# geekieo/collaborative-deep-metric-learning

Hardware: AMD Instinct MI355X
Metric: triplets/sec (higher is better)
Workload: dtype f32 values as 3 exact bf16 planes (hi + mid + lo == the f32 value), 6 bf16-MFMA plane products per f32 product, f32 accumulate

## Files before the change

__graft_entry__.py:

```python
import glob
import os
import subprocess
import sys

ROOT = os.path.dirname(os.path.abspath(__file__))
PKG = os.path.join(ROOT, "collaborative-deep-metric-learning_amd")
CSRC = os.path.join(PKG, "csrc")
LIB = os.path.join(PKG, "lib", "libcdml_hip.so")
if ROOT not in sys.path:
    sys.path.insert(0, ROOT)


def _stale(target, sources):
    if not os.path.exists(target):
        return True
    t = os.path.getmtime(target)
    return any(os.path.getmtime(s) > t for s in sources)


def _ids():
    import importlib.util
    spec = importlib.util.spec_from_file_location("_cdml_lib_ids", os.path.join(PKG, "_lib.py"))
    m = importlib.util.module_from_spec(spec)
    spec.loader.exec_module(m)
# ... 4 lines not shown
    from concurrent.futures import ThreadPoolExecutor
    os.makedirs(objdir, exist_ok=True)
    jobs = []
    import re
    for s in srcs:
        o = os.path.join(objdir, os.path.basename(s)[:-4] + ".o")
        inc = [os.path.join(os.path.dirname(s), m) for m in re.findall(r'#include "([^"]+\.hip)"', open(s).read())]
        if force or _stale(o, [s] + inc + hdrs):
            jobs.append([hipcc] + flags + ["-c", "-o", o, s])
    if jobs:
        print("[build] compiling %d of %d sources" % (len(jobs), len(srcs)), flush=True)

        def run(c):
            r = subprocess.run(c + ["-Rpass-analysis=kernel-resource-usage"], cwd=CSRC, stderr=subprocess.PIPE, text=True)
            o = c[c.index("-o") + 1]
            with open(o[:-2] + ".remarks", "w") as f:
                f.write(r.stderr)
            if r.returncode:
                sys.stderr.write("\n".join(ln for ln in r.stderr.splitlines() if "remark:" not in ln)[-4000:] + "\n")
            return r
        with ThreadPoolExecutor(max_workers=min(len(jobs), max(1, (os.cpu_count() or 2) - 1))) as ex:
            for r in ex.map(run, jobs):
                if r.returncode:
                    raise RuntimeError("hipcc failed: " + " ".join(r.args))
    objs = [os.path.join(objdir, os.path.basename(s)[:-4] + ".o") for s in srcs]
    _check_no_scratch(objs)
    return objs


NPAIR_KERNELS = ("k_npair", "k_mixed", "k_npdp")


def _check_no_scratch(objs):
    import re
    bad = []
    for o in objs:
        rem = o[:-2] + ".remarks"
        if not os.path.exists(rem):
            continue
        name = None
        for ln in open(rem):
            m = re.search(r"Function Name: (\S+)", ln)
            if m:
                name = m.group(1)
            m = re.search(r"ScratchSize \[bytes/lane\]: (\d+)", ln)
            if m and name and int(m.group(1)) > 0 and any(k in name for k in ("k_gemm",) + NPAIR_KERNELS):
                bad.append("%s: %s bytes of scratch per lane (%s)" % (name, m.group(1), os.path.basename(o)))
    if bad:
        raise RuntimeError("kernels with a scratch frame (GEMMs: spills inside hand-counted vmcnt pipelines; N-pair launches "
                           "(k_npair / k_mixed / k_npdp): spills in bandwidth-bound passes):\n  " + "\n  ".join(bad))


def build(force=False, csrc=None, lib=None, objdir=None):
    variant = csrc is not None
    csrc = csrc or CSRC
    lib = lib or LIB
    objdir = objdir or os.path.join(ROOT, "build", "obj")
    srcs = sorted(glob.glob(os.path.join(csrc, "*.hip")))
    hdrs = glob.glob(os.path.join(csrc, "*.h")) + [os.path.join(ROOT, "include", "cdml.h")] \
        + glob.glob(os.path.join(ROOT, "include", "cdml_*.h"))
    source_id, embedded_id = _ids()
    sid = source_id(csrc, os.path.join(ROOT, "include", "cdml.h"))
    if force or embedded_id(lib) != sid:
        os.makedirs(os.path.dirname(lib), exist_ok=True)
        hipcc = os.environ.get("HIPCC", "/opt/rocm/bin/hipcc")
        flags = ["--offload-arch=gfx950", "-O3", "-std=c++17", "-fPIC", "-I" + CSRC,
                 "-Wno-array-bounds"]
        objs = _compile_objects(srcs, hdrs, objdir, hipcc, flags, force)
        idsrc = os.path.join(objdir, "build_id.cpp")
        with open(idsrc, "w") as f:
            f.write('extern "C" const char *cdml_build_id(void) { return "CDML_BUILD_ID=%s"; }\n' % sid)
        subprocess.run([hipcc, "-O1", "-fPIC", "-c", "-o", idsrc[:-4] + ".o", idsrc], check=True)
        objs.append(idsrc[:-4] + ".o")
        cmd = [hipcc, "--offload-arch=gfx950", "-fPIC", "-shared", "-o", lib] + objs
        print("[build]", " ".join(cmd), flush=True)
        subprocess.run(cmd, check=True, cwd=csrc)
    if variant:
        return
    import cdml_amd
    from cdml_amd import _lib
    lib = _lib.load_library()
    assert lib.cdml_version() >= 1000
    for name in list(_lib.SIGNATURES) + list(_lib.SIGNATURES_MIXED) + list(_lib.SIGNATURES_DP) + list(_lib.SIGNATURES_BF16) \
            + list(_lib.SIGNATURES_HARDNEG):
        getattr(lib, name)
    assert lib.cdml_build_id().decode() == "CDML_BUILD_ID=" + sid
    print("[build] ok:", LIB, "version", lib.cdml_version(), lib.cdml_build_id().decode())


def smoke():
    import numpy as np
    import torch
    build()
    from cdml_amd import engine, train
    from oracle import sampler as osampler, synth as osynth, tower as otower

    dev = torch.device("cuda:0")
    N, F, H, D, B = 512, 96, 200, 32, 128
    table = engine.FeatureTable.synthetic(N, F, seed=0, device=dev)
    feats = osynth.features_philox(0, N, F, 0)
    assert np.array_equal(table.data[:, :F].cpu().numpy(), feats), "table differs"
    pairs_np = osynth.cowatch_pairs(N, 64, seed=0)
    pairs = torch.from_numpy(pairs_np).to(dev)
    idx = osampler.device_triplets_vec(pairs_np, N, 1234, 0, B)
    x = feats[idx.reshape(-1)]
    for precision in ("f32x3", "f32", "f16x2"):
        ts = train.TrainStep(table, pairs, B, hidden_size=H, output_size=D, margin=0.8, mode="uniform",
                             optimizer="adam", base_learning_rate=0.01, device=dev, precision=precision)
        W = [t.detach().cpu().numpy().copy() for t in ts.params.unpadded()]
        ts.step()
        torch.cuda.synchronize()
        assert np.array_equal(ts.idx.view(B, 3).cpu().numpy(), idx), "sampled indices differ"
        fwd, loss, grads = otower.train_step_grads(x, W, 0.8, np.float32)
        e = ts.ws.e[:, :D].cpu().numpy()
        assert np.abs(e - fwd["l2_norm"]).max() < 1e-5, "embeddings differ (%s)" % precision
        assert abs(ts.loss() - float(loss["hinge_loss"])) < 1e-5, "loss differs (%s)" % precision
        gW1 = ts.params.unpadded(grads=True)[0].cpu().numpy()
        assert np.abs(gW1 - grads["dW1"]).max() < 1e-5, "dW1 differs (%s)" % precision
        w1, _, _ = otower.adam_step(W[0], gW1, 0 * W[0], 0 * W[0], 1, 0.01)
        assert np.abs(ts.params.unpadded()[0].cpu().numpy() - w1).max() < 1e-6, "Adam update differs (%s)" % precision
        if precision == "f32x3":
            L = ts.layout
            w1t = ts.ws.W1T[:, :L.Fp].float() + ts.ws.W1T[:, L.Fp:2 * L.Fp].float() + ts.ws.W1T[:, 2 * L.Fp:].float()
            assert torch.equal(w1t, ts.params.W1.t()), "weight planes differ from the master weights"
        if precision == "f16x2":
            L, sw = ts.layout, ts.ws.scales.w1
            w1t = (ts.ws.W1T[:, :L.Fp].double() + ts.ws.W1T[:, L.Fp:2 * L.Fp].double()) / sw
            assert (w1t - ts.params.W1.t().double()).abs().max().item() <= 2.0 ** -22 * ts.params.W1.abs().max().item(), \
                "fp16 weight planes differ from the master weights"
        print("[smoke] %s ok: loss %.6f (oracle %.6f)" % (precision, ts.loss(), float(loss["hinge_loss"])))


if __name__ == "__main__":
    build(force="--force" in sys.argv)
    if "--smoke" in sys.argv:
        smoke()
```

collaborative-deep-metric-learning_amd/_lib.py:

```python
import ctypes as C
import os

_HERE = os.path.dirname(os.path.abspath(__file__))
_LIB_NAME = "libcdml_hip.so"


class CdmlError(RuntimeError):

    def __init__(self, code, message):
        super().__init__(f"cdml status {code}: {message}")
        self.code = code


def lib_path():
    return os.environ.get("CDML_LIB_PATH") or os.path.join(_HERE, "lib", _LIB_NAME)


def source_id(csrc=None, header=None):
    import glob
    import hashlib
    csrc = csrc or os.path.join(_HERE, "csrc")
    header = header or os.path.join(os.path.dirname(_HERE), "include", "cdml.h")
    files = sorted(glob.glob(os.path.join(csrc, "*.hip")) + glob.glob(os.path.join(csrc, "*.h")))
    if not files or not os.path.exists(header):
# ... 110 lines not shown
                                _p, _sz, _p]),
    "cdml_gemm_bf16_tn": (_i, [_p, _i64, _p, _i64, _i, _i, _i, _p, _i64, _p, _p, _sz, _p]),
    "cdml_sample_gather_x3": (_i, [_i, _p, _i64, _u64, _u64, _p, _i, _i64, _i64, _p, _i64, _i64, _i,
                                   _p, _p, _p, _i64, _i, _i64, _i64, _p, _p]),
    "cdml_sample_gather_h2": (_i, [_i, _p, _i64, _u64, _u64, _p, _i, _i64, _i64, _p, _i64, _i64, _i,
                                   _p, _p, _p, _i64, _i, _i64, _i64, _p, _p]),
    "cdml_gather_rows_x3": (_i, [_p, _i64, _i64, _p, _i, _i, _i, _p, _i64, _p, _p]),
    "cdml_sample_gather_x3k": (_i, [_i, _p, _i64, _u64, _u64, _p, _i, _i64, _i64, _p, _i64, _i64, _i,
                                    _p, _p, _p, _i64, _i, _i64, _i64, _p, _p, _i64, _p]),
    "cdml_split_f32_bf16x3": (_i, [_p, _i64, _i, _i, _p, _i64, _i64, _i, _p]),
    "cdml_gemm_bf16x3_workspace": (_sz, [_i, _i, _i, _i, _i]),
    "cdml_gemm_bf16x3_nt": (_i, [_i, _p, _i64, _i64, _p, _i64, _i64, _i, _i, _i, _i, _p, _i64, _i64, _p, _p, _i64, _f,
                                 _p, _p, _sz, _p]),
    "cdml_gemm_bf16x3_tn": (_i, [_p, _i64, _i64, _p, _i64, _i64, _i, _i, _i, _i, _p, _i64, _p, _f, _p, _p, _sz, _p]),
    "cdml_split_f32_f16x2": (_i, [_p, _i64, _i, _i, _p, _i64, _i64, _i, _f, _p]),
    "cdml_gemm_f16x2_workspace": (_sz, [_i, _i, _i, _i]),
    "cdml_gemm_f16x2_nt": (_i, [_i, _p, _i64, _i64, _p, _i64, _i64, _i, _i, _i, _p, _i64, _i64, _p, _p, _i64, _f, _f, _f,
                                _p, _sz, _p]),
    "cdml_gemm_f16x2_tn": (_i, [_p, _i64, _i64, _p, _i64, _i64, _i, _i, _i, _p, _i64, _f, _p, _f, _p, _sz, _p]),
    "cdml_interleave8_bf16x3": (_i, [_p, _i64, _i64, _i, _i, _p, _p]),
    "cdml_gemm_bf16x3_tnk": (_i, [_p, _i, _i, _p, _i, _i, _i, _i, _i, _p, _i64, _p, _p, _sz, _p]),
    "cdml_transpose_to_bf16": (_i, [_i, _p, _i64, _i, _i, _p, _i64, _p]),
    "cdml_cast_f32_bf16": (_i, [_p, _i64, _i, _i, _p, _i64, _p]),
    "cdml_colsum_workspace_floats": (_sz, [_i, _i]),
    "cdml_colsum": (_i, [_i, _p, _i64, _i, _i, _p, _p, _p]),
    "cdml_fill_uniform_table_f16": (_i, [_p, _i64, _i64, _i, _i64, _u64, _p]),
    "cdml_gather_rows_f16": (_i, [_p, _i64, _i64, _i64, _p, _i, _i, _p, _i64, _p, _p]),
    "cdml_ew_combine": (_i, [_i, _p, _i64, _p, _i64, _i, _i, _p, _i64, _p]),
    "cdml_ew_fusion_bwd": (_i, [_i, _p, _i64, _p, _i64, _p, _i64, _i, _i, _f, _p, _i64, _p, _i64, _p]),
    "cdml_lrelu_bwd": (_i, [_p, _i64, _p, _i64, _i, _i, _f, _p, _i64, _p]),
    "cdml_adam_step": (_i, [_p, _p, _p, _p, _i64, _f, _p, _f, _f, _f, _i64, _p, _i, _p, _p]),
    "cdml_adam_matrix_bf16": (_i, [_p, _p, _p, _p, _i, _i, _f, _p, _f, _f, _f, _i64, _p, _p, _i64, _p, _i64,
                                   _p, _p, _p, _p, _i, _i, _p, _p]),
    "cdml_adam_matrix_planes": (_i, [_p, _p, _p, _p, _i, _i, _f, _p, _f, _f, _f, _i64, _p, _p, _i64, _i64, _p, _i64, _i64,
                                     _p, _p, _p, _p, _i, _i, _p, _p]),
    "cdml_adam_matrix_h2": (_i, [_p, _p, _p, _p, _i, _i, _f, _p, _f, _f, _f, _i64, _p, _p, _i64, _i64, _p, _i64, _i64, _f,
                                 _p, _p, _p, _p, _i, _i, _p, _p]),
    "cdml_table_adam_rows": (_i, [_p, _i64, _i64, _i64, _i, _p, _i, _p, _i64, _p, _p, _p, _p, _f, _f, _p, _f, _f, _f,
                                  _i64, _p, _p]),
    "cdml_grad_prepare": (_i, [_p, _p, _i64, _f, _f, _p, _p, _p]),
    "cdml_momentum_step": (_i, [_p, _p, _p, _i64, _f, _p, _f, _i, _p]),
    "cdml_lars_scratch_floats": (_sz, []),
    "cdml_lars_step": (_i, [_p, _p, _p, _i64, _f, _p, _f, _f, _f, _f, _p, _p]),
    "cdml_lars_multi_scratch_floats": (_sz, []),
    "cdml_lars_multi": (_i, [_p, _p, _p, _p, _p, _i, _f, _p, _f, _f, _f, _f, _p, _p, _p, _p, _p]),
    "cdml_lars_multi_norms": (_i, [_p, _p, _p, _p, _i, _p, _p]),
    "cdml_lars_matrix": (_i, [_p, _p, _p, _p, _p, _i, _i, _i, _i, _i, _f, _p, _f, _f, _f, _f, _p, _p, _p, _i64, _i64, _p,
                              _i64, _i64, _i, _p, _p, _p]),
    "cdml_momentum_matrix": (_i, [_p, _p, _p, _i, _i, _f, _p, _f, _i, _p, _i64, _i64, _p, _i64, _i64, _i, _p, _p, _p, _i,
                                  _p, _p, _p]),
    "cdml_lars_matrix_h2": (_i, [_p, _p, _p, _p, _p, _i, _i, _i, _i, _i, _f, _p, _f, _f, _f, _f, _p, _p, _p, _i64, _i64, _p,
                                 _i64, _i64, _f, _p, _p, _p]),
    "cdml_momentum_matrix_h2": (_i, [_p, _p, _p, _i, _i, _f, _p, _f, _i, _p, _i64, _i64, _p, _i64, _i64, _f, _p, _p, _p, _i,
                                     _p, _p, _p]),
}

SIGNATURES_MIXED = {
    "cdml_npair_mixed_workspace": (_sz, [_i, _i]),
    "cdml_npair_mixed_stats": (_i, [_p, _i64, _p, _i, _i64, _i64, _p, _i, _p, _f, _p, _f, _i, _p, _p, _p, _sz, _p]),
    "cdml_npair_mixed_grad_x3": (_i, [_p, _i64, _p, _i, _i64, _i64, _p, _i, _p, _f, _p, _f, _i, _p, _p, _i64, _i64, _p]),
    "cdml_npair_mixed_grad_f32": (_i, [_p, _i64, _p, _i, _i64, _i64, _p, _i, _p, _f, _p, _f, _i, _p, _p, _i64, _p]),
    "cdml_npair_mixed_split_x3": (_i, [_p, _i64, _i, _i, _p, _i64, _i64, _p, _i64, _i64, _p, _i64, _i64, _i64, _p]),
}

SIGNATURES_DP = {
    "cdml_npair_dp_workspace": (_sz, [_i, _i]),
    "cdml_npair_dp_local_stats": (_i, [_p, _i64, _p, _i, _i, _i, _f, _i, _p, _p, _p, _sz, _p]),
    "cdml_npair_dp_col_fold": (_i, [_p, _i, _i, _p, _p]),
    "cdml_npair_dp_stats": (_i, [_p, _i64, _i, _i, _i, _f, _i, _p, _p, _p, _sz, _p]),
    "cdml_npair_dp_grad_x3": (_i, [_p, _i64, _p, _i, _i, _i, _f, _i, _p, _p, _p, _i64, _i64, _p]),
    "cdml_npair_dp_grad_f32": (_i, [_p, _i64, _p, _i, _i, _i, _f, _i, _p, _p, _p, _i64, _p]),
    "cdml_npair_dp_pos_fold": (_i, [_p, _i64, _i, _i, _i, _p, _i64, _p]),
}

SIGNATURES_BF16 = {
    "cdml_npair_operands_bf16": (_i, [_p, _i64, _i, _i, _p, _i64, _p, _i64, _p, _i64, _p]),
    "cdml_npair_grad_bf16": (_i, [_p, _i64, _p, _i, _f, _i, _p, _p, _i64, _p]),
    "cdml_npair_logq_grad_bf16": (_i, [_p, _i64, _p, _i, _p, _f, _i, _p, _p, _i64, _p]),
    "cdml_npair_memory_grad_bf16": (_i, [_p, _i64, _p, _i, _i64, _p, _i, _f, _i, _p, _p, _i64, _p]),
    "cdml_npair_memory_logq_grad_bf16": (_i, [_p, _i64, _p, _i, _i64, _p, _p, _i, _f, _i, _p, _p, _i64, _p]),
    "cdml_npair_memory_push_bf16": (_i, [_p, _i64, _p, _i, _i, _u64, _p, _i64, _i, _p, _i64, _p, _p, _i64, _p, _i64, _p]),
}

SIGNATURES_HARDNEG = {
    "cdml_sample_listed": (_i, [_p, _i64, _i64, _u64, _u64, _p, _i, _i64, _i64, _p, _i64, _i, _u64, _p, _p, _p]),
    "cdml_sample_gather_listed": (_i, [_p, _i64, _u64, _u64, _p, _i, _i64, _i64, _p, _i64, _i64, _i, _p, _i64, _i, _u64,
                                       _p, _p, _p, _i64, _i, _i64, _i64, _i64, _p, _p]),
    "cdml_sample_gather_listed_x3": (_i, [_p, _i64, _u64, _u64, _p, _i, _i64, _i64, _p, _i64, _i64, _i, _p, _i64, _i, _u64,
                                          _p, _p, _p, _i64, _i, _i64, _i64, _i64, _p, _p, _i64, _p]),
    "cdml_sample_gather_listed_f16": (_i, [_p, _i64, _u64, _u64, _p, _i, _i64, _i64, _p, _i64, _i64, _i, _p, _i64, _i, _u64,
                                           _p, _p, _p, _i64, _i, _i64, _i64, _i64, _p, _p]),
}

_lib = None


def load_library():
    global _lib
    if _lib is not None:
        return _lib
    path = lib_path()
    if not os.path.exists(path):
        raise CdmlError(-2, f"{path} not found: build it with "
                            f"`python -c 'import __graft_entry__ as g; g.build()'` "
                            f"(there is no CPU fallback)")
    import torch
    lib = C.CDLL(path)
    for name, (res, args) in (list(SIGNATURES.items()) + list(SIGNATURES_MIXED.items()) + list(SIGNATURES_DP.items())
                               + list(SIGNATURES_BF16.items()) + list(SIGNATURES_HARDNEG.items())):
        fn = getattr(lib, name)
        fn.restype = res
        fn.argtypes = args
    want = source_id()
    if want is not None and not os.environ.get("CDML_LIB_PATH") and os.environ.get("CDML_ALLOW_STALE_LIB") != "1":
        have = lib.cdml_build_id().decode()
        if have != "CDML_BUILD_ID=" + want:
            raise CdmlError(-2, f"{path} was built from other sources ({have}; this tree is {want}): rebuild it with "
                                f"`python -c 'import __graft_entry__ as g; g.build()'`")
    _lib = lib
    return lib


def call(name, *args):
    lib = load_library()
    rc = getattr(lib, name)(*args)
    if rc != 0:
        raise CdmlError(rc, lib.cdml_last_error().decode("utf-8", "replace"))
    return rc
```

collaborative-deep-metric-learning_amd/csrc/gemm_bf16x3.hip:

```cpp
#include "gemm_bf16.h"
#include <stdlib.h>

namespace cdml {
namespace {

using bf16x4 = __attribute__((ext_vector_type(4))) __bf16;
using f32x4 = __attribute__((ext_vector_type(4))) float;
constexpr int kThreads = 256;

__device__ __forceinline__ void split3(float v, bf16 &h, bf16 &m, bf16 &l) {
  h = (bf16)v;
  const float r = v - (float)h;
  m = (bf16)r;
  l = (bf16)(r - (float)m);
}

__global__ void __launch_bounds__(kThreads)
k_split3(const float *__restrict__ src, int64_t lds_, int rows, int cols, bf16 *__restrict__ dst, int64_t ldd,
         int64_t plane) {
  const int c4n = cols >> 2;
  const int64_t total = (int64_t)rows * c4n;
  for (int64_t i = (int64_t)blockIdx.x * blockDim.x + threadIdx.x; i < total; i += (int64_t)gridDim.x * blockDim.x) {
    const int64_t r = i / c4n;
    const int c = (int)(i - r * c4n) * 4;
    const f32x4 v = *reinterpret_cast<const f32x4 *>(src + r * lds_ + c);
    bf16x4 h, m, l;
#pragma unroll
    for (int j = 0; j < 4; ++j) {
      bf16 a, b, c_;
      split3(v[j], a, b, c_);
      h[j] = a; m[j] = b; l[j] = c_;
    }
    bf16 *d = dst + r * ldd + c;
    *reinterpret_cast<bf16x4 *>(d) = h;
    *reinterpret_cast<bf16x4 *>(d + plane) = m;
    *reinterpret_cast<bf16x4 *>(d + 2 * plane) = l;
  }
}

__global__ void __launch_bounds__(kThreads)
k_split3_transpose(const float *__restrict__ src, int64_t lds_, int rows, int cols, bf16 *__restrict__ dst,
                   int64_t ldd, int64_t plane) {
  __shared__ float tile[64][65];
  const int r0 = blockIdx.y * 64, c0 = blockIdx.x * 64;
  const int tx = threadIdx.x & 63, ty = threadIdx.x >> 6;
  for (int j = ty; j < 64; j += 4) {
    const int r = r0 + j, c = c0 + tx;
    tile[j][tx] = (r < rows && c < cols) ? src[(int64_t)r * lds_ + c] : 0.f;
  }
  __syncthreads();
  for (int j = ty; j < 64; j += 4) {
    const int c = c0 + j, r = r0 + tx;
    if (c < cols && r < rows) {
      bf16 h, m, l;
      split3(tile[tx][j], h, m, l);
      bf16 *d = dst + (int64_t)c * ldd + r;
      d[0] = h; d[plane] = m; d[2 * plane] = l;
    }
  }
}

using half4v = __attribute__((ext_vector_type(4))) _Float16;
__device__ __forceinline__ void split2h(float v, float scale, _Float16 &h, _Float16 &l) {
  const float s = __builtin_amdgcn_fmed3f(v * scale, -65504.f, 65504.f);
  h = (_Float16)s;
  l = (_Float16)(s - (float)h);
}

__global__ void __launch_bounds__(kThreads)
k_split2h(const float *__restrict__ src, int64_t lds_, int rows, int cols, _Float16 *__restrict__ dst, int64_t ldd,
          int64_t plane, float scale) {
  const int c4n = cols >> 2;
  const int64_t total = (int64_t)rows * c4n;
  for (int64_t i = (int64_t)blockIdx.x * blockDim.x + threadIdx.x; i < total; i += (int64_t)gridDim.x * blockDim.x) {
    const int64_t r = i / c4n;
    const int c = (int)(i - r * c4n) * 4;
    const f32x4 v = *reinterpret_cast<const f32x4 *>(src + r * lds_ + c);
    half4v h, l;
#pragma unroll
    for (int j = 0; j < 4; ++j) {
      _Float16 a, b;
      split2h(v[j], scale, a, b);
      h[j] = a; l[j] = b;
// ... 107 lines not shown
  tl_slab_steps = steps >= 12 ? steps / 6 * 6 : 0;
  return prev;
}

extern "C" size_t cdml_gemm_bf16x3_workspace(int tn, int M, int N, int K, int products) {
  if (M <= 0 || N <= 0 || K <= 0 || (products != 3 && products != 6) || K % 64) return 0;
  const int ktiles = products * (K / 64);
  int requested = tn ? gemm_bf16_256_splits(M, N, ktiles * 64) : x3_nt_splits(N, ktiles, (M + 255) / 256);
  if (!tn && N / 256 == 1) {
    const int s60 = ktiles / 60 < 1 ? 1 : (ktiles / 60 > 16 ? 16 : ktiles / 60);
    if (s60 > requested) requested = s60;
  }
  int splits = requested, per = 0, s2 = requested;
  x3_split_geometry(ktiles, requested, products == 6 ? 6 : 2, per, splits);
  x3_split_geometry(ktiles, requested, 2, per, s2);
  if (s2 > splits) splits = s2;
  const size_t cs = (size_t)splits * ((M + 255) / 256) * 2 * N * sizeof(float) + (size_t)N * sizeof(float);
  return (size_t)splits * M * N * sizeof(float) + cs;
}

extern "C" size_t cdml_gemm_f16x2_workspace(int tn, int M, int N, int K) {
  const size_t a = cdml_gemm_bf16x3_workspace(tn, M, N, K, 6), b = cdml_gemm_bf16x3_workspace(tn, M, N, K, 3);
  return a > b ? a : b;
}

namespace cdml {
namespace {
__device__ __forceinline__ void x3_colsum_block(const float *__restrict__ partial, int n_rows, int N, float *__restrict__ out,
                                                int blk, float scale) {
  __shared__ float red[16][17];
  const int cl = threadIdx.x & 15, rl = threadIdx.x >> 4;
  const int c = blk * 16 + cl;
  float s0 = 0.f, s1 = 0.f, s2 = 0.f, s3 = 0.f;
  if (c < N) {
    int r = rl;
    for (; r + 48 < n_rows; r += 64) {
      s0 += partial[(int64_t)r * N + c];
      s1 += partial[(int64_t)(r + 16) * N + c];
      s2 += partial[(int64_t)(r + 32) * N + c];
      s3 += partial[(int64_t)(r + 48) * N + c];
    }
    for (; r < n_rows; r += 16) s0 += partial[(int64_t)r * N + c];
  }
  red[rl][cl] = (s0 + s1) + (s2 + s3);
  __syncthreads();
  if (rl == 0 && c < N) {
    float t = red[0][cl];
#pragma unroll
    for (int j = 1; j < 16; ++j) t += red[j][cl];
    out[c] = t * scale;
  }
}

__global__ void __launch_bounds__(kThreads)
k_x3_sum_slabs(const float *__restrict__ slabs, int64_t slab_stride, int splits, int rows, int N,
               const float *__restrict__ bias, float alpha, float *__restrict__ out, int64_t ldo, int slab_blocks,
               const float *__restrict__ cs_partial, int cs_rows, float *__restrict__ cs_out, float cs_scale) {
  if ((int)blockIdx.x >= slab_blocks) {
    x3_colsum_block(cs_partial, cs_rows, N, cs_out, blockIdx.x - slab_blocks, cs_scale);
    return;
  }
  const int n4 = N >> 2;
  const int64_t total = (int64_t)rows * n4;
  for (int64_t i = (int64_t)blockIdx.x * blockDim.x + threadIdx.x; i < total; i += (int64_t)slab_blocks * blockDim.x) {
    const int64_t r = i / n4;
    const int c = (int)(i - r * n4);
    f32x4 s = reinterpret_cast<const f32x4 *>(slabs)[i];
    for (int z = 1; z < splits; ++z) s += reinterpret_cast<const f32x4 *>(slabs + (int64_t)z * slab_stride)[i];
    if (bias) {
      s += reinterpret_cast<const f32x4 *>(bias)[c];
      s.x = fmaxf(s.x, s.x * alpha); s.y = fmaxf(s.y, s.y * alpha);
      s.z = fmaxf(s.z, s.z * alpha); s.w = fmaxf(s.w, s.w * alpha);
    }
    reinterpret_cast<f32x4 *>(out + r * ldo)[c] = s;
  }
}
}
}

static int gemm_x3_nt_impl(bool f16, float out_scale, float c_scale, int epilogue, const uint16_t *A, int64_t lda, int64_t plane_a,
                           const uint16_t *B, int64_t ldb, int64_t plane_b, int M, int N, int K, int products, void *C,
                           int64_t ldc, int64_t plane_c, const float *bias, const uint16_t *aux,
                           int64_t ldaux, float alpha, float *colsum, void *workspace,
                           size_t workspace_bytes, cdml_stream_t stream) {
  CDML_REQUIRE(A && B && C && M > 0 && N > 0 && K > 0, CDML_E_BADARG, "gemm_bf16x3_nt: bad argument");
  const int np1 = f16 ? 1 : 2;
  CDML_REQUIRE(!f16 || (products == 3 && epilogue != BE_MASKBITS_X3_KI && epilogue != BE_ROWBIAS_LRELU_X3 && !colsum &&
                        out_scale > 0.f && c_scale > 0.f),
               CDML_E_UNSUPPORTED, "gemm_f16x2_nt: epilogues 1, 3, 6, 7, 9, 10, positive scales, no column sums");
  const bool kint_out = epilogue == BE_MASKBITS_X3_KI;
  const bool bits_out = epilogue == BE_BIAS_LRELU_X3_BITS, bits_in = epilogue == BE_MASKBITS_X3 || (kint_out && aux);
  if (bits_out) epilogue = BE_BIAS_LRELU_X3;
  if (bits_in || kint_out) epilogue = BE_MASK_X3;
  CDML_REQUIRE(epilogue == BE_BIAS_LRELU_F32 || epilogue == BE_F32 || epilogue == BE_BIAS_LRELU_X3 || epilogue == BE_MASK_X3 ||
                   epilogue == BE_ROWBIAS_LRELU_X3,
               CDML_E_BADARG, "gemm_bf16x3_nt: epilogue must be 1, 3, 6, 7, 8, 9, 10 or 12");
  CDML_REQUIRE(!(bits_out || bits_in) || (aux && N % 8 == 0 && ldaux >= N / 8), CDML_E_BADARG,
               "gemm_bf16x3_nt: epilogues 9 / 10 need the bitmask in aux (ldaux >= N / 8 bytes)");
  CDML_REQUIRE(products == 3 || products == 6, CDML_E_BADARG, "gemm_bf16x3_nt: products must be 3 or 6");
  CDML_REQUIRE(N % 256 == 0 && K % 64 == 0, CDML_E_UNSUPPORTED,
               "gemm_bf16x3_nt: N must be a multiple of 256 and K of 64, got N=%d K=%d", N, K);
  CDML_REQUIRE(aligned16(A) && aligned16(B) && aligned16(C) && !(lda & 7) && !(ldb & 7) && !(plane_a & 7) && !(plane_b & 7) &&
                   plane_a >= K && plane_b >= K && lda >= np1 * plane_a + K && ldb >= np1 * plane_b + K,
               CDML_E_ALIGN, "gemm_bf16x3_nt: 16-B aligned bases, strides multiples of 8, ld >= 2 plane + K (fp16 form: plane + K)");
  const bool planes_out = epilogue == BE_BIAS_LRELU_X3 || epilogue == BE_MASK_X3 || epilogue == BE_ROWBIAS_LRELU_X3;
  CDML_REQUIRE(kint_out ? (M % 8 == 0 && !(ldc & 7) && ldc >= N && plane_c >= (int64_t)(M / 8) * ldc * 8 &&
                           (int64_t)3 * plane_c * 2 < ((int64_t)1 << 32))
                        : planes_out ? (!(ldc & 7) && !(plane_c & 7) && plane_c >= N && ldc >= np1 * plane_c + N) : (!(ldc & 3) && ldc >= N),
               CDML_E_ALIGN, "gemm_bf16x3_nt: ldc (plane outputs: ldc and plane_c multiples of 8, ldc >= 2 plane_c + N; epilogue 12: M a "
               "multiple of 8, ldc = columns per row group >= N, plane_c >= M ldc)");
  CDML_REQUIRE(epilogue != BE_MASK_X3 || !aux || bits_in || (aligned16(aux) && !(ldaux & 7) && ldaux >= N), CDML_E_ALIGN,
               "gemm_bf16x3_nt: aux must be 16-B aligned with ldaux a multiple of 8");
  CDML_REQUIRE((epilogue != BE_BIAS_LRELU_F32 && epilogue != BE_BIAS_LRELU_X3 && epilogue != BE_ROWBIAS_LRELU_X3) || bias,
               CDML_E_BADARG, "gemm_bf16x3_nt: bias required");
  CDML_REQUIRE(!colsum || (M % 256 == 0 && products == 6 && epilogue == BE_F32), CDML_E_UNSUPPORTED,
               "gemm_bf16x3_nt: colsum (sum over k of B[n][k]) goes with epilogue 3, M a multiple of 256 and six products");
  CDML_REQUIRE(((int64_t)M + 256) * lda * 2 < ((int64_t)1 << 31) && (int64_t)N * ldb * 2 < ((int64_t)1 << 31), CDML_E_UNSUPPORTED,
               "gemm_bf16x3_nt: an operand exceeds the 2 GiB buffer-descriptor range");
  BArgs g{};
  g.A = reinterpret_cast<const bf16 *>(A); g.lda = lda;
  g.B = reinterpret_cast<const bf16 *>(B); g.ldb = ldb;
  g.C = C; g.ldc = ldc; g.bias = bias; g.alpha = alpha;
  g.aux = reinterpret_cast<const bf16 *>(aux); g.ldaux = ldaux;
  if (bits_out) { g.mask_out = reinterpret_cast<uint8_t *>(const_cast<uint16_t *>(aux)); g.ldmask = ldaux; g.aux = nullptr; g.ldaux = 0; }
  g.aux_bits = bits_in ? 1 : 0;
  g.c_kint = kint_out ? 1 : 0;
  g.M = M; g.N = N;
  g.x3_tpp = K / 64; g.x3_plane_a = plane_a; g.x3_plane_b = plane_b; g.x3_plane_c = plane_c;
  g.x3_products = (f16 || x3_kmajor()) ? products : 0;
  g.out_scale = out_scale; g.c_scale = c_scale;
  const int ktiles = products * g.x3_tpp;
  CDML_REQUIRE(ktiles % 2 == 0, CDML_E_UNSUPPORTED, "gemm_bf16x3_nt: products * K / 64 must be even");
  g.K = ktiles * 64; g.k_per_split = g.K;
  g.tiles_m = (M + 255) / 256; g.tiles_n = N / 256;
  hipStream_t s = (hipStream_t)stream;
  auto launch = [&](int epi, int n_splits) {
    return f16 ? launch_gemm_f16x2_256(g, false, epi, n_splits, s) : launch_gemm_bf16_256_x3(g, false, epi, n_splits, s);
  };
  int splits = planes_out ? 1 : x3_nt_splits(N, ktiles, g.tiles_m, f16), per = ktiles;
  if (splits > 1) x3_split_geometry(ktiles, splits, 6, per, splits);
  if (splits > 1) {
    if (!workspace) {
      splits = 1;
    } else {
      const size_t need = (size_t)splits * M * N * sizeof(float) + (colsum ? (size_t)splits * g.tiles_m * 2 * N * sizeof(float) : 0);
      CDML_REQUIRE(workspace_bytes >= need && aligned16(workspace), CDML_E_BADARG,
                   "gemm_bf16x3_nt: the slab form needs a 16-B aligned workspace of %zu bytes (cdml_gemm_bf16x3_workspace); pass "
                   "NULL for the single-pass form", need);
    }
  }
  const size_t slab_bytes = splits > 1 ? (size_t)splits * M * N * sizeof(float) : 0;
  const size_t cs_rows = (size_t)splits * g.tiles_m * 2;
  if (colsum) {
    CDML_REQUIRE(workspace && aligned16(workspace) && workspace_bytes >= slab_bytes + cs_rows * N * sizeof(float), CDML_E_BADARG,
                 "gemm_bf16x3_nt: colsum needs a workspace (cdml_gemm_bf16x3_workspace)");
    g.colsum_partial = reinterpret_cast<float *>(static_cast<char *>(workspace) + slab_bytes);
  }
  int rc;
  if (splits == 1) {
    rc = launch(epilogue, 1);
  } else {
    g.k_per_split = per * 64;
    g.slab_stride = (int64_t)M * N;
    g.C = workspace; g.ldc = N;
    rc = launch(BE_F32, splits);
    if (rc) return rc;
    const int sb = grid1d((int64_t)M * N / 4), cb = colsum ? (N + 15) / 16 : 0;
    hipLaunchKernelGGL(k_x3_sum_slabs, dim3(sb + cb), dim3(kThreads), 0, s,
                       static_cast<const float *>(workspace), g.slab_stride, splits, M, N,
                       epilogue == BE_BIAS_LRELU_F32 ? bias : nullptr, alpha, static_cast<float *>(C), ldc, sb,
                       g.colsum_partial, (int)cs_rows, colsum, 1.0f);
    return check_launch("gemm_bf16x3_nt combine");
  }
  if (rc || !colsum) return rc;
  hipLaunchKernelGGL(k_x3_sum_slabs, dim3((N + 15) / 16), dim3(kThreads), 0, s, static_cast<const float *>(nullptr), (int64_t)0, 0, 0,
                     N, static_cast<const float *>(nullptr), 0.f, static_cast<float *>(nullptr), (int64_t)0, 0, g.colsum_partial,
                     (int)cs_rows, colsum, 1.0f);
  return check_launch("gemm_bf16x3_nt bias gradient");
}

extern "C" int cdml_gemm_bf16x3_nt(int epilogue, const uint16_t *A, int64_t lda, int64_t plane_a, const uint16_t *B,
                                   int64_t ldb, int64_t plane_b, int M, int N, int K, int products, void *C,
                                   int64_t ldc, int64_t plane_c, const float *bias, const uint16_t *aux,
                                   int64_t ldaux, float alpha, float *colsum, void *workspace,
                                   size_t workspace_bytes, cdml_stream_t stream) {
  return gemm_x3_nt_impl(false, 1.0f, 1.0f, epilogue, A, lda, plane_a, B, ldb, plane_b, M, N, K, products, C, ldc, plane_c, bias, aux,
                         ldaux, alpha, colsum, workspace, workspace_bytes, stream);
}

extern "C" int cdml_gemm_f16x2_nt(int epilogue, const uint16_t *A, int64_t lda, int64_t plane_a, const uint16_t *B,
                                  int64_t ldb, int64_t plane_b, int M, int N, int K, void *C, int64_t ldc, int64_t plane_c,
                                  const float *bias, const uint16_t *aux, int64_t ldaux, float alpha, float out_scale,
                                  float c_scale, void *workspace, size_t workspace_bytes, cdml_stream_t stream) {
  return gemm_x3_nt_impl(true, out_scale, c_scale, epilogue, A, lda, plane_a, B, ldb, plane_b, M, N, K, 3, C, ldc, plane_c, bias, aux,
                         ldaux, alpha, nullptr, workspace, workspace_bytes, stream);
}

static int gemm_x3_tn_impl(bool f16, float out_scale, float cs_scale, const uint16_t *A, int64_t lda, int64_t plane_a,
                           const uint16_t *B, int64_t ldb, int64_t plane_b, int M, int N, int K, int products, float *C, int64_t ldc,
                           const float *bias, float alpha, float *colsum, void *workspace,
                           size_t workspace_bytes, cdml_stream_t stream) {
  CDML_REQUIRE(A && B && C && M > 0 && N > 0 && K > 0, CDML_E_BADARG, "gemm_bf16x3_tn: bad argument");
  const int np1 = f16 ? 1 : 2;
  CDML_REQUIRE(!f16 || (products == 3 && out_scale > 0.f && cs_scale > 0.f), CDML_E_BADARG, "gemm_f16x2_tn: positive scales");
  CDML_REQUIRE(products == 3 || products == 6, CDML_E_BADARG, "gemm_bf16x3_tn: products must be 3 or 6");
  CDML_REQUIRE(M % 256 == 0 && N % 256 == 0 && K % 128 == 0, CDML_E_UNSUPPORTED,
               "gemm_bf16x3_tn: M, N must be multiples of 256 and K of 128, got M=%d N=%d K=%d", M, N, K);
  CDML_REQUIRE(aligned16(A) && aligned16(B) && aligned16(C) && !(lda & 7) && !(ldb & 7) && !(plane_a & 7) && !(plane_b & 7) &&
                   !(ldc & 3) && plane_a >= M && plane_b >= N && lda >= np1 * plane_a + M && ldb >= np1 * plane_b + N && ldc >= N,
               CDML_E_ALIGN, "gemm_bf16x3_tn: 16-B aligned bases, strides multiples of 8, ld >= 2 plane + columns");
  CDML_REQUIRE((int64_t)K * lda * 2 < ((int64_t)1 << 31) && (int64_t)K * ldb * 2 < ((int64_t)1 << 31), CDML_E_UNSUPPORTED,
               "gemm_bf16x3_tn: an operand exceeds the 2 GiB buffer-descriptor range");
  BArgs g{};
  g.A = reinterpret_cast<const bf16 *>(A); g.lda = lda;
  g.B = reinterpret_cast<const bf16 *>(B); g.ldb = ldb;
  g.M = M; g.N = N;
  g.x3_tpp = K / 64; g.x3_plane_a = plane_a; g.x3_plane_b = plane_b;
  g.x3_products = (f16 || x3_kmajor()) ? products : 0;
  g.out_scale = out_scale; g.c_scale = 1.0f;
  const int ktiles = products * g.x3_tpp;
  g.K = ktiles * 64;
  g.tiles_m = M / 256; g.tiles_n = N / 256;
  int splits = gemm_bf16_256_splits(M, N, g.K), per = 0;
  x3_split_geometry(ktiles, splits, ((products == 6 && g.x3_products == 6) || f16) ? 6 : 2, per, splits);
  const bool slabs = splits > 1 || bias != nullptr;
  const size_t slab_bytes = slabs ? (size_t)splits * M * N * sizeof(float) : 0;
  const size_t cs_rows = (size_t)splits * g.tiles_m * 2;
  const size_t need = slab_bytes + (colsum ? cs_rows * N * sizeof(float) : 0);
  CDML_REQUIRE(need == 0 || (workspace && workspace_bytes >= need && aligned16(workspace)), CDML_E_BADARG,
               "gemm_bf16x3_tn: workspace of %zu bytes required (cdml_gemm_bf16x3_workspace)", need);
  hipStream_t s = (hipStream_t)stream;
  g.k_per_split = per * 64;
  g.slab_stride = (int64_t)M * N;
  g.C = slabs ? workspace : static_cast<void *>(C);
  g.ldc = slabs ? N : ldc;
  g.colsum_partial = colsum ? reinterpret_cast<float *>(static_cast<char *>(workspace) + slab_bytes) : nullptr;
  int rc = f16 ? launch_gemm_f16x2_256(g, true, BE_F32, splits, s) : launch_gemm_bf16_256_x3(g, true, BE_F32, splits, s);
  if (rc) return rc;
  if (slabs || colsum) {
    const int sb = slabs ? grid1d((int64_t)M * N / 4) : 0, cb = colsum ? (N + 15) / 16 : 0;
    hipLaunchKernelGGL(k_x3_sum_slabs, dim3(sb + cb), dim3(kThreads), 0, s, static_cast<const float *>(workspace), g.slab_stride,
                       splits, M, N, bias, alpha, C, ldc, sb, g.colsum_partial, (int)cs_rows, colsum, cs_scale);
    rc = check_launch("gemm_bf16x3_tn combine");
  }
  return rc;
}

extern "C" int cdml_gemm_bf16x3_tn(const uint16_t *A, int64_t lda, int64_t plane_a, const uint16_t *B, int64_t ldb,
                                   int64_t plane_b, int M, int N, int K, int products, float *C, int64_t ldc,
                                   const float *bias, float alpha, float *colsum, void *workspace,
                                   size_t workspace_bytes, cdml_stream_t stream) {
  return gemm_x3_tn_impl(false, 1.0f, 1.0f, A, lda, plane_a, B, ldb, plane_b, M, N, K, products, C, ldc, bias, alpha, colsum, workspace,
                         workspace_bytes, stream);
}

extern "C" int cdml_gemm_f16x2_tn(const uint16_t *A, int64_t lda, int64_t plane_a, const uint16_t *B, int64_t ldb,
                                  int64_t plane_b, int M, int N, int K, float *C, int64_t ldc, float out_scale, float *colsum,
                                  float colsum_scale, void *workspace, size_t workspace_bytes, cdml_stream_t stream) {
  return gemm_x3_tn_impl(true, out_scale, colsum_scale, A, lda, plane_a, B, ldb, plane_b, M, N, K, 3, C, ldc, nullptr, 0.f, colsum,
                         workspace, workspace_bytes, stream);
}

namespace cdml {
namespace {

__global__ void __launch_bounds__(kThreads)
k_mine_prep(const float *__restrict__ e_in, float *__restrict__ e_out, int64_t lde, const float *__restrict__ z, int64_t ldz,
            int B, int D, bf16 *__restrict__ e3, int64_t ld3, int64_t plane, float *__restrict__ sqn, float *__restrict__ dp,
            float h2_scale) {
  const int lane = threadIdx.x & 63, wave = threadIdx.x >> 6;
// ... 247 lines not shown
```

collaborative-deep-metric-learning_amd/csrc/loss.hip:

```cpp
#include "common.h"

namespace cdml {
namespace {

constexpr int kThreads = 256;
constexpr int kWavesPerBlock = kThreads / kWave;
constexpr float kL2Eps = 1e-12f;

__device__ __forceinline__ float4 ld4(const float *p, int q) {
  return reinterpret_cast<const float4 *>(p)[q];
}
__device__ __forceinline__ void st4(float *p, int q, float4 v) {
  reinterpret_cast<float4 *>(p)[q] = v;
}
__device__ __forceinline__ float sq4(float4 a) { return a.x * a.x + a.y * a.y + a.z * a.z + a.w * a.w; }
__device__ __forceinline__ float dot4(float4 a, float4 b) { return a.x * b.x + a.y * b.y + a.z * b.z + a.w * b.w; }
__device__ __forceinline__ float4 sub4(float4 a, float4 b) { return make_float4(a.x - b.x, a.y - b.y, a.z - b.z, a.w - b.w); }
__device__ __forceinline__ float4 mul4(float4 a, float s) { return make_float4(a.x * s, a.y * s, a.z * s, a.w * s); }

__global__ void __launch_bounds__(kThreads)
k_l2norm_fwd(const float *__restrict__ x, int64_t ldx, int M, int N, float *__restrict__ y,
             int64_t ldy, float *__restrict__ inv_out) {
  const int lane = threadIdx.x & (kWave - 1);
  const int wave = threadIdx.x >> 6;
  const int nq = N >> 2;
  for (int r = blockIdx.x * kWavesPerBlock + wave; r < M; r += gridDim.x * kWavesPerBlock) {
    const float *xr = x + (int64_t)r * ldx;
    float ss = 0.f;
    for (int q = lane; q < nq; q += kWave) ss += sq4(ld4(xr, q));
    ss = wave_sum(ss);
    const float inv = 1.0f / sqrtf(fmaxf(ss, kL2Eps));
    if (inv_out && lane == 0) inv_out[r] = inv;
    float *yr = y + (int64_t)r * ldy;
    for (int q = lane; q < nq; q += kWave) st4(yr, q, mul4(ld4(xr, q), inv));
  }
}

__global__ void __launch_bounds__(kThreads)
k_l2norm_bwd(const float *__restrict__ z, int64_t ldz, const float *__restrict__ g, int64_t ldg,
             int M, int N, float alpha, float *__restrict__ dz, int64_t lddz) {
  const int lane = threadIdx.x & (kWave - 1);
  const int wave = threadIdx.x >> 6;
  const int nq = N >> 2;
  for (int r = blockIdx.x * kWavesPerBlock + wave; r < M; r += gridDim.x * kWavesPerBlock) {
    const float *zr = z + (int64_t)r * ldz;
    const float *gr = g + (int64_t)r * ldg;
    float ss = 0.f, zg = 0.f;
    for (int q = lane; q < nq; q += kWave) {
      const float4 a = ld4(zr, q);
      ss += sq4(a);
      zg += dot4(a, ld4(gr, q));
    }
    ss = wave_sum(ss);
    zg = wave_sum(zg);
    const float inv = 1.0f / sqrtf(fmaxf(ss, kL2Eps));
    const float c = (ss > kL2Eps) ? inv * inv * zg : 0.f;
    float *dr = dz + (int64_t)r * lddz;
    for (int q = lane; q < nq; q += kWave) {
      const float4 a = ld4(zr, q), b = ld4(gr, q);
      float4 d = make_float4(inv * (b.x - a.x * c), inv * (b.y - a.y * c), inv * (b.z - a.z * c),
                             inv * (b.w - a.w * c));
      if (alpha >= 0.f) {
        d.x *= (a.x > 0.f) ? 1.f : alpha;
        d.y *= (a.y > 0.f) ? 1.f : alpha;
        d.z *= (a.z > 0.f) ? 1.f : alpha;
        d.w *= (a.w > 0.f) ? 1.f : alpha;
      }
      st4(dr, q, d);
    }
  }
}

__device__ __forceinline__ void dist_pair(const float *a, const float *p, const float *n, int nq,
                                          int lane, float &pos, float &neg) {
  float sp = 0.f, sn = 0.f;
  for (int q = lane; q < nq; q += kWave) {
    const float4 va = ld4(a, q);
    sp += sq4(sub4(va, ld4(p, q)));
    sn += sq4(sub4(va, ld4(n, q)));
  }
  pos = wave_sum(sp);
  neg = wave_sum(sn);
}
// ... 11 lines not shown
    float pos, neg;
    dist_pair(a, p, n, nq, lane, pos, neg);
    const float t = pos - neg + margin;
    if (lane == 0) {
      pos_o[i] = pos;
      neg_o[i] = neg;
      hinge_o[i] = fmaxf(t, 0.f);
    }
    if (de) {
      const float s = (t >= 0.f) ? two_over_b : 0.f;
      float *da = de + (int64_t)(3 * i) * ldde, *dp = da + ldde, *dn = dp + ldde;
      for (int q = lane; q < nq; q += kWave) {
        const float4 va = ld4(a, q), vp = ld4(p, q), vn = ld4(n, q);
        st4(da, q, mul4(sub4(vn, vp), s));
        st4(dp, q, mul4(sub4(vp, va), s));
        st4(dn, q, mul4(sub4(va, vn), s));
      }
    }
  }
}

__global__ void __launch_bounds__(kThreads)
k_triplet_hinge_inbatch(const float *__restrict__ e, int64_t lde, const int32_t *__restrict__ rows,
                        const int32_t *__restrict__ shift_p, int B, int D, float margin,
                        float *__restrict__ pos_o, float *__restrict__ neg_o,
                        float *__restrict__ hinge_o, uint8_t *__restrict__ valid_o,
                        float *__restrict__ de, int64_t ldde) {
  const int lane = threadIdx.x & (kWave - 1);
  const int wave = threadIdx.x >> 6;
  const int nq = D >> 2;
  const int shift = *shift_p;
  const float two_over_b = 2.0f / (float)B;
  for (int i = blockIdx.x * kWavesPerBlock + wave; i < B; i += gridDim.x * kWavesPerBlock) {
    const int j = (i + shift) % B;
    const int k = (i - shift % B + B) % B;
    const float *a = e + (int64_t)(2 * i) * lde, *p = a + lde;
    const float *n = e + (int64_t)(2 * j + 1) * lde;
    const int32_t va_id = rows[2 * i], vp_id = rows[2 * i + 1], vn_id = rows[2 * j + 1];
    const bool valid_i = (vn_id != va_id) && (vn_id != vp_id);
    float pos, neg;
    dist_pair(a, p, n, nq, lane, pos, neg);
    const float t = pos - neg + margin;
    if (lane == 0) {
      pos_o[i] = pos;
      neg_o[i] = neg;
      hinge_o[i] = valid_i ? fmaxf(t, 0.f) : 0.f;
      if (valid_o) valid_o[i] = valid_i ? 1 : 0;
    }
    if (de) {
      const float *ak = e + (int64_t)(2 * k) * lde, *pk = ak + lde;
      const bool valid_k = (vp_id != rows[2 * k]) && (vp_id != rows[2 * k + 1]);
      float posk, negk;
      dist_pair(ak, pk, p, nq, lane, posk, negk);
      const float si = (valid_i && t >= 0.f) ? two_over_b : 0.f;
      const float sk = (valid_k && (posk - negk + margin) >= 0.f) ? two_over_b : 0.f;
      float *da = de + (int64_t)(2 * i) * ldde, *dp = da + ldde;
      for (int q = lane; q < nq; q += kWave) {
        const float4 va = ld4(a, q), vp = ld4(p, q), vn = ld4(n, q), vak = ld4(ak, q);
        st4(da, q, mul4(sub4(vn, vp), si));
        const float4 g1 = mul4(sub4(vp, va), si);
        const float4 g2 = mul4(sub4(vak, vp), sk);
        st4(dp, q, make_float4(g1.x + g2.x, g1.y + g2.y, g1.z + g2.z, g1.w + g2.w));
      }
    }
  }
}

template <int NCH>
struct TailRow {
  float4 v[NCH];
  float ss, inv;
  __device__ __forceinline__ void load(const float *zr, int nq, int lane) {
    float s = 0.f;
#pragma unroll
    for (int c = 0; c < NCH; ++c) {
      const int q = lane + kWave * c;
      v[c] = (q < nq) ? ld4(zr, q) : make_float4(0.f, 0.f, 0.f, 0.f);
      s += sq4(v[c]);
    }
    ss = wave_sum(s);
    inv = 1.0f / sqrtf(fmaxf(ss, kL2Eps));
  }
  __device__ __forceinline__ float4 e(int c) const { return mul4(v[c], inv); }
};

template <int NCH>
__device__ __forceinline__ void tail_dist(const TailRow<NCH> &a, const TailRow<NCH> &p, const TailRow<NCH> &n,
                                          float &pos, float &neg) {
  float sp = 0.f, sn = 0.f;
#pragma unroll
  for (int c = 0; c < NCH; ++c) {
    const float4 va = a.e(c);
    sp += sq4(sub4(va, p.e(c)));
    sn += sq4(sub4(va, n.e(c)));
  }
  pos = wave_sum(sp);
  neg = wave_sum(sn);
}

template <int NCH>
__device__ __forceinline__ void tail_store_row(const TailRow<NCH> &r, const float4 (&g)[NCH], float alpha,
                                               float *er, float *dr, uint16_t *br, int nq, int lane,
                                               int64_t plane = 0, float h2_scale = 0.f) {
  float zg = 0.f;
#pragma unroll
  for (int c = 0; c < NCH; ++c) zg += dot4(r.v[c], g[c]);
  zg = wave_sum(zg);
  const float inv = r.inv;
  const float cc = (r.ss > kL2Eps) ? inv * inv * zg : 0.f;
#pragma unroll
  for (int c = 0; c < NCH; ++c) {
    const int q = lane + kWave * c;
    if (q >= nq) continue;
    const float4 a = r.v[c], b = g[c];
    float4 d = make_float4(inv * (b.x - a.x * cc), inv * (b.y - a.y * cc), inv * (b.z - a.z * cc),
                           inv * (b.w - a.w * cc));
    if (alpha >= 0.f) {
      d.x *= (a.x > 0.f) ? 1.f : alpha;
      d.y *= (a.y > 0.f) ? 1.f : alpha;
      d.z *= (a.z > 0.f) ? 1.f : alpha;
      d.w *= (a.w > 0.f) ? 1.f : alpha;
    }
    st4(er, q, r.e(c));
    st4(dr, q, d);
    if (br && h2_scale > 0.f) {
      using half4v = __attribute__((ext_vector_type(4))) _Float16;
      const float dv[4] = {d.x, d.y, d.z, d.w};
      half4v hi, lo;
#pragma unroll
      for (int u = 0; u < 4; ++u) {
        const float sv = __builtin_amdgcn_fmed3f(dv[u] * h2_scale, -65504.f, 65504.f);
        hi[u] = (_Float16)sv;
        lo[u] = (_Float16)(sv - (float)hi[u]);
      }
      reinterpret_cast<half4v *>(br)[q] = hi;
      reinterpret_cast<half4v *>(br + plane)[q] = lo;
    } else if (br) {
      auto rn = [](float x) -> uint32_t {
        const uint32_t u = __float_as_uint(x);
        return (u + 0x7fffu + ((u >> 16) & 1u)) >> 16;
      };
      uint2 w;
      w.x = rn(d.x) | (rn(d.y) << 16);
      w.y = rn(d.z) | (rn(d.w) << 16);
      reinterpret_cast<uint2 *>(br)[q] = w;
      if (plane) {
        float r[4] = {d.x, d.y, d.z, d.w};
        uint32_t hb[4] = {w.x & 0xffffu, w.x >> 16, w.y & 0xffffu, w.y >> 16};
#pragma unroll
        for (int pl = 1; pl < 3; ++pl) {
#pragma unroll
          for (int u = 0; u < 4; ++u) {
            r[u] -= __uint_as_float(hb[u] << 16);
            hb[u] = rn(r[u]);
          }
          uint2 m;
          m.x = hb[0] | (hb[1] << 16);
          m.y = hb[2] | (hb[3] << 16);
          reinterpret_cast<uint2 *>(br + pl * plane)[q] = m;
        }
      }
    }
  }
}

template <int MODE, int NCH>
__global__ void __launch_bounds__(kThreads)
k_vnet_tail(const float *__restrict__ z, int64_t ldz, const int32_t *__restrict__ rows,
            const int32_t *__restrict__ shift_p, int B, int D, float margin, float alpha,
            float *__restrict__ e, int64_t lde, float *__restrict__ pos_o, float *__restrict__ neg_o,
            float *__restrict__ hinge_o, uint8_t *__restrict__ valid_o, float *__restrict__ dz2,
            int64_t lddz, uint16_t *__restrict__ dz2_bf, int64_t ldbf, float *__restrict__ var_ws,
            int64_t plane_bf, float h2_scale) {
  __shared__ __attribute__((aligned(16))) float s_red[kWavesPerBlock][8];
  extern __shared__ __attribute__((aligned(16))) float s_col[];
  const int lane = threadIdx.x & (kWave - 1);
  const int wave = threadIdx.x >> 6;
  const int nq = D >> 2;
  const int shift = (MODE == 1) ? *shift_p : 0;
  const float two_over_b = 2.0f / (float)B;
  float4 csum[NCH];
  float tsq = 0.f;
#pragma unroll
  for (int c = 0; c < NCH; ++c) csum[c] = make_float4(0.f, 0.f, 0.f, 0.f);
  for (int i = blockIdx.x * kWavesPerBlock + wave; i < B; i += gridDim.x * kWavesPerBlock) {
    TailRow<NCH> A, P, N;
    float4 ga[NCH], gp[NCH];
    int64_t ra, rp;
    bool valid_i = true;
    float pos, neg;
    if (MODE == 0) {
      ra = 3 * (int64_t)i; rp = ra + 1;
      A.load(z + ra * ldz, nq, lane);
      P.load(z + rp * ldz, nq, lane);
      N.load(z + (ra + 2) * ldz, nq, lane);
      tail_dist<NCH>(A, P, N, pos, neg);
      const float t = pos - neg + margin;
      const float s = (t >= 0.f) ? two_over_b : 0.f;
      float4 gn[NCH];
#pragma unroll
      for (int c = 0; c < NCH; ++c) {
        const float4 va = A.e(c), vp = P.e(c), vn = N.e(c);
        ga[c] = mul4(sub4(vn, vp), s);
        gp[c] = mul4(sub4(vp, va), s);
        gn[c] = mul4(sub4(va, vn), s);
      }
      if (lane == 0) { pos_o[i] = pos; neg_o[i] = neg; hinge_o[i] = fmaxf(t, 0.f); }
      tail_store_row<NCH>(N, gn, alpha, e + (ra + 2) * lde, dz2 + (ra + 2) * lddz,
                          dz2_bf ? dz2_bf + (ra + 2) * ldbf : nullptr, nq, lane, plane_bf, h2_scale);
    } else {
      const int j = (i + shift) % B;
      const int k = (i - shift % B + B) % B;
      ra = 2 * (int64_t)i; rp = ra + 1;
      const int32_t va_id = rows[2 * i], vp_id = rows[2 * i + 1], vn_id = rows[2 * j + 1];
      valid_i = (vn_id != va_id) && (vn_id != vp_id);
      const bool valid_k = (vp_id != rows[2 * k]) && (vp_id != rows[2 * k + 1]);
      TailRow<NCH> AK, PK;
      A.load(z + ra * ldz, nq, lane);
      P.load(z + rp * ldz, nq, lane);
      N.load(z + (int64_t)(2 * j + 1) * ldz, nq, lane);
      AK.load(z + (int64_t)(2 * k) * ldz, nq, lane);
      PK.load(z + (int64_t)(2 * k + 1) * ldz, nq, lane);
      tail_dist<NCH>(A, P, N, pos, neg);
      float posk, negk;
      tail_dist<NCH>(AK, PK, P, posk, negk);
      const float t = pos - neg + margin;
      const float si = (valid_i && t >= 0.f) ? two_over_b : 0.f;
      const float sk = (valid_k && (posk - negk + margin) >= 0.f) ? two_over_b : 0.f;
#pragma unroll
      for (int c = 0; c < NCH; ++c) {
        const float4 va = A.e(c), vp = P.e(c), vn = N.e(c), vak = AK.e(c);
        ga[c] = mul4(sub4(vn, vp), si);
        const float4 g1 = mul4(sub4(vp, va), si);
        const float4 g2 = mul4(sub4(vak, vp), sk);
        gp[c] = make_float4(g1.x + g2.x, g1.y + g2.y, g1.z + g2.z, g1.w + g2.w);
      }
      if (lane == 0) {
        pos_o[i] = pos; neg_o[i] = neg;
        hinge_o[i] = valid_i ? fmaxf(t, 0.f) : 0.f;
        if (valid_o) valid_o[i] = valid_i ? 1 : 0;
      }
    }
    tail_store_row<NCH>(A, ga, alpha, e + ra * lde, dz2 + ra * lddz, dz2_bf ? dz2_bf + ra * ldbf : nullptr, nq, lane, plane_bf, h2_scale);
    tail_store_row<NCH>(P, gp, alpha, e + rp * lde, dz2 + rp * lddz, dz2_bf ? dz2_bf + rp * ldbf : nullptr, nq, lane, plane_bf, h2_scale);
    if (var_ws) {
#pragma unroll
      for (int c = 0; c < NCH; ++c) {
        const float4 va = A.e(c), vp = P.e(c), vn = N.e(c);
        csum[c].x += va.x + vp.x + vn.x; csum[c].y += va.y + vp.y + vn.y;
        csum[c].z += va.z + vp.z + vn.z; csum[c].w += va.w + vp.w + vn.w;
        tsq += sq4(va) + sq4(vp) + sq4(vn);
      }
    }
  }
  if (!var_ws) return;
  float *mine = s_col + wave * D;
#pragma unroll
  for (int c = 0; c < NCH; ++c) {
    const int q = lane + kWave * c;
    if (q < nq) st4(mine, q, csum[c]);
  }
  tsq = wave_sum(tsq);
  if (lane == 0) s_red[wave][0] = tsq;
  __syncthreads();
  float *out = var_ws + (int64_t)blockIdx.x * (D + 4);
  for (int d = threadIdx.x; d < D; d += kThreads) {
    float v = 0.f;
    for (int w = 0; w < kWavesPerBlock; ++w) v += s_col[w * D + d];
    out[d] = v;
  }
  if (threadIdx.x == 0) {
    float v = 0.f;
    for (int w = 0; w < kWavesPerBlock; ++w) v += s_red[w][0];
    out[D] = v;
  }
}

__global__ void __launch_bounds__(kThreads)
k_tail_var_final(const float *__restrict__ var_ws, int nb, int B, int D, float *__restrict__ stats) {
  __shared__ double s_v[kWavesPerBlock];
  const int lane = threadIdx.x & (kWave - 1), wave = threadIdx.x >> 6;
  const double n_rows = 3.0 * (double)B;
  double vsum = 0.0;
  for (int d = threadIdx.x; d < D; d += kThreads) {
    double col = 0.0;
    for (int b = 0; b < nb; ++b) col += (double)var_ws[(int64_t)b * (D + 4) + d];
    const double mean = col / n_rows;
    vsum -= n_rows * mean * mean;
  }
  for (int b = threadIdx.x; b < nb; b += kThreads) vsum += (double)var_ws[(int64_t)b * (D + 4) + D];
#pragma unroll
  for (int off = 32; off > 0; off >>= 1) vsum += __shfl_xor(vsum, off, 64);
  if (lane == 0) s_v[wave] = vsum;
  __syncthreads();
  if (threadIdx.x == 0) {
    double v = 0.0;
    for (int w = 0; w < kWavesPerBlock; ++w) v += s_v[w];
    stats[4] = (float)(v / (n_rows * (double)D));
  }
}

__global__ void __launch_bounds__(kThreads)
k_row_sumsq(const float *__restrict__ e, int64_t lde, int R, int D, float *__restrict__ sqn) {
  const int lane = threadIdx.x & (kWave - 1);
  const int wave = threadIdx.x >> 6;
  const int nq = D >> 2;
  for (int r = blockIdx.x * kWavesPerBlock + wave; r < R; r += gridDim.x * kWavesPerBlock) {
    float ss = 0.f;
    for (int q = lane; q < nq; q += kWave) ss += sq4(ld4(e + (int64_t)r * lde, q));
    ss = wave_sum(ss);
    if (lane == 0) sqn[r] = ss;
  }
}

struct Cand { float d; int c; };
__device__ __forceinline__ bool closer(float d, int c, const Cand &b) {
  return d < b.d || (d == b.d && c < b.c);
}
__device__ __forceinline__ bool farther(float d, int c, const Cand &b) {
  return d > b.d || (d == b.d && c < b.c);
}

__global__ void __launch_bounds__(kThreads)
k_semihard_select(const float *__restrict__ S, int64_t ldS, const float *__restrict__ sqn,
                  const int32_t *__restrict__ rows, int B, int32_t *__restrict__ neg_row) {
  const int lane = threadIdx.x & (kWave - 1);
  const int wave = threadIdx.x >> 6;
  const int R = 2 * B;
  const float inf = __builtin_huge_valf();
  for (int i = blockIdx.x * kWavesPerBlock + wave; i < B; i += gridDim.x * kWavesPerBlock) {
    const float *Si = S + (int64_t)i * ldS;
    const float sa = sqn[2 * i];
    const int32_t va = rows[2 * i], vp = rows[2 * i + 1];
    const float dp = sa + sqn[2 * i + 1] - 2.0f * Si[2 * i + 1];
    Cand out{inf, 0x7fffffff}, in{-inf, 0x7fffffff};
    auto scan4 = [&](int q, const float4 s4, const int4 r4, const float4 n4) {
      const float sv[4] = {s4.x, s4.y, s4.z, s4.w};
      const int32_t rv[4] = {r4.x, r4.y, r4.z, r4.w};
      const float nv[4] = {n4.x, n4.y, n4.z, n4.w};
#pragma unroll
      for (int u = 0; u < 4; ++u) {
        const int c = 4 * q + u;
        if (rv[u] != va && rv[u] != vp) {
          const float d = sa + nv[u] - 2.0f * sv[u];
          if (d > dp) { if (closer(d, c, out)) out = Cand{d, c}; }
          if (farther(d, c, in)) in = Cand{d, c};
        }
      }
    };
    const int nq = R >> 2;
    const int4 *rows4 = reinterpret_cast<const int4 *>(rows);
    int q = lane;
    for (; q + 3 * kWave < nq; q += 4 * kWave) {
      float4 sv[4], nv[4];
      int4 rv[4];
#pragma unroll
      for (int u = 0; u < 4; ++u) {
        using f32x4 = __attribute__((ext_vector_type(4))) float;
        const f32x4 t4 = __builtin_nontemporal_load(reinterpret_cast<const f32x4 *>(Si) + q + u * kWave);
        sv[u] = make_float4(t4.x, t4.y, t4.z, t4.w);
        rv[u] = rows4[q + u * kWave];
        nv[u] = ld4(sqn, q + u * kWave);
      }
#pragma unroll
      for (int u = 0; u < 4; ++u) scan4(q + u * kWave, sv[u], rv[u], nv[u]);
    }
    for (; q < nq; q += kWave) scan4(q, ld4(Si, q), rows4[q], ld4(sqn, q));
#pragma unroll
    for (int off = 32; off > 0; off >>= 1) {
      const float od = __shfl_xor(out.d, off, 64); const int oc = __shfl_xor(out.c, off, 64);
      if (closer(od, oc, out)) out = Cand{od, oc};
      const float id = __shfl_xor(in.d, off, 64); const int ic = __shfl_xor(in.c, off, 64);
      if (farther(id, ic, in)) in = Cand{id, ic};
    }
    if (lane == 0) neg_row[i] = (out.c != 0x7fffffff) ? out.c : (in.c != 0x7fffffff ? in.c : -1);
  }
}

__global__ void __launch_bounds__(kThreads)
k_hinge_indexed_fwd(const float *__restrict__ e, int64_t lde, const int32_t *__restrict__ neg_row,
                    int B, int D, float margin, float *__restrict__ pos_o, float *__restrict__ neg_o,
                    float *__restrict__ hinge_o, float *__restrict__ scale) {
// ... 325 lines not shown
int grid_rows(int rows) {
  int64_t b = ((int64_t)rows + kWavesPerBlock - 1) / kWavesPerBlock;
  if (b > kNumCU * 8) b = kNumCU * 8;
  return (int)(b < 1 ? 1 : b);
}

int check_rows(const char *who, const void *p, int64_t ld, int N) {
  CDML_REQUIRE(p, CDML_E_BADARG, "%s: null pointer", who);
  CDML_REQUIRE((N & 3) == 0 && ld >= N && (ld & 3) == 0 && aligned16(p), CDML_E_ALIGN,
               "%s: width and leading dimension must be multiples of 4, base 16-B aligned", who);
  return CDML_OK;
}

}
}

using namespace cdml;

extern "C" int cdml_l2norm_fwd(const float *x, int64_t ldx, int M, int N, float *y, int64_t ldy,
                               float *inv_out, cdml_stream_t stream) {
  CDML_REQUIRE(M > 0 && N > 0, CDML_E_BADARG, "l2norm_fwd: bad shape");
  int rc;
  if ((rc = check_rows("l2norm_fwd", x, ldx, N))) return rc;
  if ((rc = check_rows("l2norm_fwd", y, ldy, N))) return rc;
  hipLaunchKernelGGL(k_l2norm_fwd, dim3(grid_rows(M)), dim3(kThreads), 0, (hipStream_t)stream, x, ldx,
                     M, N, y, ldy, inv_out);
  return check_launch("l2norm_fwd");
}

extern "C" int cdml_l2norm_bwd(const float *z, int64_t ldz, const float *g, int64_t ldg, int M, int N,
                               float lrelu_alpha, float *dz, int64_t lddz, cdml_stream_t stream) {
  CDML_REQUIRE(M > 0 && N > 0, CDML_E_BADARG, "l2norm_bwd: bad shape");
  int rc;
  if ((rc = check_rows("l2norm_bwd", z, ldz, N))) return rc;
  if ((rc = check_rows("l2norm_bwd", g, ldg, N))) return rc;
  if ((rc = check_rows("l2norm_bwd", dz, lddz, N))) return rc;
  hipLaunchKernelGGL(k_l2norm_bwd, dim3(grid_rows(M)), dim3(kThreads), 0, (hipStream_t)stream, z, ldz,
                     g, ldg, M, N, lrelu_alpha, dz, lddz);
  return check_launch("l2norm_bwd");
}

extern "C" int cdml_triplet_hinge(const float *e, int64_t lde, int B, int D, float margin, float *pos,
                                  float *neg, float *hinge, float *stats, float *de, int64_t ldde,
                                  cdml_stream_t stream) {
  CDML_REQUIRE(B > 0 && D > 0 && pos && neg && hinge, CDML_E_BADARG, "triplet_hinge: bad argument");
  int rc;
  if ((rc = check_rows("triplet_hinge", e, lde, D))) return rc;
  if (de && (rc = check_rows("triplet_hinge", de, ldde, D))) return rc;
  hipLaunchKernelGGL(k_triplet_hinge, dim3(grid_rows(B)), dim3(kThreads), 0, (hipStream_t)stream, e,
                     lde, B, D, margin, pos, neg, hinge, de, ldde);
  if ((rc = check_launch("triplet_hinge"))) return rc;
  if (stats) {
    hipLaunchKernelGGL(k_loss_stats, dim3(1), dim3(1024), 0, (hipStream_t)stream, pos, neg, hinge, B,
                       stats);
    rc = check_launch("triplet_hinge stats");
  }
  return rc;
}

extern "C" int cdml_triplet_hinge_inbatch(const float *e, int64_t lde, const int32_t *rows,
                                          const int32_t *shift, int B, int D, float margin,
                                          float *pos, float *neg, float *hinge, uint8_t *valid_out,
                                          float *stats, float *de, int64_t ldde,
                                          cdml_stream_t stream) {
  CDML_REQUIRE(B >= 2 && D > 0 && rows && shift && pos && neg && hinge, CDML_E_BADARG,
               "triplet_hinge_inbatch: bad argument");
  int rc;
  if ((rc = check_rows("triplet_hinge_inbatch", e, lde, D))) return rc;
  if (de && (rc = check_rows("triplet_hinge_inbatch", de, ldde, D))) return rc;
  hipLaunchKernelGGL(k_triplet_hinge_inbatch, dim3(grid_rows(B)), dim3(kThreads), 0,
                     (hipStream_t)stream, e, lde, rows, shift, B, D, margin, pos, neg, hinge,
                     valid_out, de, ldde);
  if ((rc = check_launch("triplet_hinge_inbatch"))) return rc;
  if (stats) {
    hipLaunchKernelGGL(k_loss_stats, dim3(1), dim3(1024), 0, (hipStream_t)stream, pos, neg, hinge, B,
                       stats);
    rc = check_launch("triplet_hinge_inbatch stats");
  }
  return rc;
}

constexpr int kTailVarBlocks = 256;

extern "C" size_t cdml_vnet_tail_workspace(int B, int D) {
  if (B <= 0 || D <= 0) return 0;
  return (size_t)kTailVarBlocks * (size_t)(D + 4) * sizeof(float);
}

static int vnet_tail_impl(int mode, const float *z, int64_t ldz, const int32_t *rows,
                          const int32_t *shift, int B, int D, float margin, float lrelu_alpha,
                          float *e, int64_t lde, float *pos, float *neg, float *hinge,
                          uint8_t *valid_out, float *dz2, int64_t lddz2, uint16_t *dz2_bf16,
                          int64_t ldbf, int64_t plane_bf, float *stats, float *var_ws, cdml_stream_t stream,
                          float h2_scale = 0.f) {
  CDML_REQUIRE(mode == 0 || mode == 1, CDML_E_BADARG, "vnet_tail: mode must be 0 (a,p,n rows) or 1 (in-batch)");
  CDML_REQUIRE(B >= (mode == 1 ? 2 : 1) && D > 0 && pos && neg && hinge, CDML_E_BADARG, "vnet_tail: bad argument");
  CDML_REQUIRE(mode == 0 || (rows && shift), CDML_E_BADARG, "vnet_tail: in-batch mode needs rows and shift");
  CDML_REQUIRE(!var_ws || stats, CDML_E_BADARG, "vnet_tail: the variance is written to stats[4]");
  CDML_REQUIRE(D <= 1024, CDML_E_UNSUPPORTED, "vnet_tail: embedding size %d > 1024", D);
  int rc;
  if ((rc = check_rows("vnet_tail z", z, ldz, D))) return rc;
  if ((rc = check_rows("vnet_tail e", e, lde, D))) return rc;
  if ((rc = check_rows("vnet_tail dz2", dz2, lddz2, D))) return rc;
  CDML_REQUIRE(!dz2_bf16 || (ldbf >= D && (ldbf & 3) == 0 && (reinterpret_cast<uintptr_t>(dz2_bf16) & 7) == 0),
               CDML_E_ALIGN, "vnet_tail: bf16 copy needs an 8-B aligned base and a leading dimension multiple of 4");
  CDML_REQUIRE(plane_bf == 0 || (dz2_bf16 && plane_bf >= D && (plane_bf & 3) == 0 && ldbf >= (h2_scale > 0.f ? 1 : 2) * plane_bf + D),
               CDML_E_ALIGN, "vnet_tail: planes need plane >= D (a multiple of 4) and a leading dimension >= 2 plane + D (fp16 planes: plane + D)");
  int grid = grid_rows(B);
  if (var_ws && grid > kTailVarBlocks) grid = kTailVarBlocks;
  const size_t lds = var_ws ? (size_t)kWavesPerBlock * D * sizeof(float) : 0;
  const int nch = ((D >> 2) + kWave - 1) / kWave;
#define CDML_LAUNCH_TAIL(M, N)                                                                       \
  hipLaunchKernelGGL((k_vnet_tail<M, N>), dim3(grid), dim3(kThreads), lds, (hipStream_t)stream, z, ldz, \
                     rows, shift, B, D, margin, lrelu_alpha, e, lde, pos, neg, hinge, valid_out, dz2,  \
                     lddz2, dz2_bf16, ldbf, var_ws, plane_bf, h2_scale)
  if (mode == 0) {
    if (nch <= 1) CDML_LAUNCH_TAIL(0, 1); else if (nch <= 2) CDML_LAUNCH_TAIL(0, 2); else CDML_LAUNCH_TAIL(0, 4);
  } else {
    if (nch <= 1) CDML_LAUNCH_TAIL(1, 1); else if (nch <= 2) CDML_LAUNCH_TAIL(1, 2); else CDML_LAUNCH_TAIL(1, 4);
  }
#undef CDML_LAUNCH_TAIL
  if ((rc = check_launch("vnet_tail"))) return rc;
  if (stats) {
    hipLaunchKernelGGL(k_loss_stats, dim3(1), dim3(1024), 0, (hipStream_t)stream, pos, neg, hinge, B, stats);
    if ((rc = check_launch("vnet_tail stats"))) return rc;
  }
  if (var_ws) {
    hipLaunchKernelGGL(k_tail_var_final, dim3(1), dim3(kThreads), 0, (hipStream_t)stream, var_ws, grid, B, D, stats);
    rc = check_launch("vnet_tail variance");
  }
  return rc;
}

extern "C" int cdml_vnet_tail(int mode, const float *z, int64_t ldz, const int32_t *rows,
                              const int32_t *shift, int B, int D, float margin, float lrelu_alpha,
                              float *e, int64_t lde, float *pos, float *neg, float *hinge,
                              uint8_t *valid_out, float *dz2, int64_t lddz2, uint16_t *dz2_bf16,
                              int64_t ldbf, float *stats, float *var_ws, cdml_stream_t stream) {
  return vnet_tail_impl(mode, z, ldz, rows, shift, B, D, margin, lrelu_alpha, e, lde, pos, neg, hinge, valid_out, dz2, lddz2,
                        dz2_bf16, ldbf, 0, stats, var_ws, stream);
}

extern "C" int cdml_vnet_tail_planes(int mode, const float *z, int64_t ldz, const int32_t *rows,
                                     const int32_t *shift, int B, int D, float margin, float lrelu_alpha,
                                     float *e, int64_t lde, float *pos, float *neg, float *hinge,
                                     uint8_t *valid_out, float *dz2, int64_t lddz2, uint16_t *dz2_planes,
                                     int64_t ldbf, int64_t plane_bf, float *stats, float *var_ws,
                                     cdml_stream_t stream) {
  CDML_REQUIRE(dz2_planes && plane_bf > 0, CDML_E_BADARG, "vnet_tail_planes: the plane buffer and its plane stride are required");
  return vnet_tail_impl(mode, z, ldz, rows, shift, B, D, margin, lrelu_alpha, e, lde, pos, neg, hinge, valid_out, dz2, lddz2,
                        dz2_planes, ldbf, plane_bf, stats, var_ws, stream);
}

extern "C" int cdml_vnet_tail_h2(int mode, const float *z, int64_t ldz, const int32_t *rows,
                                 const int32_t *shift, int B, int D, float margin, float lrelu_alpha,
                                 float *e, int64_t lde, float *pos, float *neg, float *hinge,
                                 uint8_t *valid_out, float *dz2, int64_t lddz2, uint16_t *dz2_planes,
                                 int64_t ldbf, int64_t plane_h, float scale, float *stats, float *var_ws,
                                 cdml_stream_t stream) {
  CDML_REQUIRE(dz2_planes && plane_h > 0 && scale > 0.f, CDML_E_BADARG, "vnet_tail_h2: the plane buffer, its plane stride and a positive scale are required");
  return vnet_tail_impl(mode, z, ldz, rows, shift, B, D, margin, lrelu_alpha, e, lde, pos, neg, hinge, valid_out, dz2, lddz2,
                        dz2_planes, ldbf, plane_h, stats, var_ws, stream, scale);
}

extern "C" int cdml_semihard_select(const float *S, int64_t ldS, const float *e, int64_t lde,
                                    const int32_t *rows, int B, int D, float *sqn_scratch,
                                    int32_t *neg_row_out, cdml_stream_t stream) {
  CDML_REQUIRE(B >= 1 && D > 0 && rows && sqn_scratch && neg_row_out, CDML_E_BADARG,
               "semihard_select: bad argument");
  int rc;
  if ((rc = check_rows("semihard_select e", e, lde, D))) return rc;
  if ((rc = check_rows("semihard_select S", S, ldS, 2 * B))) return rc;
  CDML_REQUIRE(aligned16(rows) && aligned16(sqn_scratch), CDML_E_ALIGN,
               "semihard_select: rows and sqn_scratch must be 16-B aligned");
  hipLaunchKernelGGL(k_row_sumsq, dim3(grid_rows(2 * B)), dim3(kThreads), 0, (hipStream_t)stream, e,
                     lde, 2 * B, D, sqn_scratch);
  hipLaunchKernelGGL(k_semihard_select, dim3(grid_rows(B)), dim3(kThreads), 0, (hipStream_t)stream, S,
                     ldS, sqn_scratch, rows, B, neg_row_out);
  return check_launch("semihard_select");
}

extern "C" int cdml_triplet_hinge_indexed_tail(const float *e, int64_t lde, const int32_t *neg_row, int B, int D,
                                               float margin, float *pos, float *neg, float *hinge, float *stats,
                                               float *scale_scratch, float *de, int64_t ldde, const float *z,
                                               int64_t ldz, float lrelu_alpha, float *dz2, int64_t lddz,
                                               uint16_t *dz2_bf16, int64_t ldbf, int64_t plane_bf,
                                               cdml_stream_t stream) {
  CDML_REQUIRE(B >= 1 && D > 0 && neg_row && pos && neg && hinge && scale_scratch, CDML_E_BADARG,
               "triplet_hinge_indexed: bad argument");
  int rc;
  if ((rc = check_rows("triplet_hinge_indexed", e, lde, D))) return rc;
  if (de && (rc = check_rows("triplet_hinge_indexed", de, ldde, D))) return rc;
  CDML_REQUIRE(!de || (aligned16(neg_row) && aligned16(scale_scratch)), CDML_E_ALIGN,
               "triplet_hinge_indexed: neg_row and scale_scratch must be 16-B aligned");
  if (z) {
    CDML_REQUIRE(de && dz2, CDML_E_BADARG, "triplet_hinge_indexed_tail: the fused tail needs de and dz2");
    if ((rc = check_rows("triplet_hinge_indexed_tail z", z, ldz, D))) return rc;
    if ((rc = check_rows("triplet_hinge_indexed_tail dz2", dz2, lddz, D))) return rc;
    CDML_REQUIRE(!dz2_bf16 || ((reinterpret_cast<uintptr_t>(dz2_bf16) & 7) == 0 && (ldbf & 3) == 0 && (plane_bf & 3) == 0 &&
                               ldbf >= (plane_bf ? 2 * plane_bf + D : D) && plane_bf >= 0),
                 CDML_E_ALIGN, "triplet_hinge_indexed_tail: dz2_bf16 8-B aligned, ldbf and plane_bf multiples of 4, ldbf >= 2 plane_bf + D");
  }
  hipStream_t s = (hipStream_t)stream;
  hipLaunchKernelGGL(k_hinge_indexed_fwd, dim3(grid_rows(B)), dim3(kThreads), 0, s, e, lde, neg_row, B,
                     D, margin, pos, neg, hinge, scale_scratch);
  if (de) {
    const int nch = ((D >> 2) + kWave - 1) / kWave;
    CDML_REQUIRE(nch <= 4, CDML_E_UNSUPPORTED, "triplet_hinge_indexed: embeddings of at most 1024 dimensions (got %d)", D);
    const dim3 grid((2 * B + kIdxRows - 1) / kIdxRows);
#define CDML_LAUNCH_HIB(N)                                                                                          \
    hipLaunchKernelGGL((k_hinge_indexed_bwd<N>), grid, dim3(kThreads), 0, s, e, lde, neg_row, scale_scratch, B, D, de, \
                       ldde, z, ldz, lrelu_alpha, dz2, lddz, dz2_bf16, ldbf, plane_bf)
    if (nch <= 1) CDML_LAUNCH_HIB(1);
    else if (nch == 2) CDML_LAUNCH_HIB(2);
    else CDML_LAUNCH_HIB(4);
#undef CDML_LAUNCH_HIB
  }
  if ((rc = check_launch("triplet_hinge_indexed"))) return rc;
  if (stats) {
    hipLaunchKernelGGL(k_loss_stats, dim3(1), dim3(1024), 0, s, pos, neg, hinge, B, stats);
    rc = check_launch("triplet_hinge_indexed stats");
  }
  return rc;
}

extern "C" int cdml_triplet_hinge_indexed(const float *e, int64_t lde, const int32_t *neg_row, int B,
                                          int D, float margin, float *pos, float *neg, float *hinge,
                                          float *stats, float *scale_scratch, float *de, int64_t ldde,
                                          cdml_stream_t stream) {
  return cdml_triplet_hinge_indexed_tail(e, lde, neg_row, B, D, margin, pos, neg, hinge, stats, scale_scratch, de, ldde,
                                         nullptr, 0, -1.0f, nullptr, 0, nullptr, 0, 0, stream);
}

extern "C" int cdml_pair_dist(const float *e, int64_t lde, int n_rows, const int32_t *pairs, int P,
// ... 60 lines not shown
```

collaborative-deep-metric-learning_amd/engine_x3.py:

```python
import os

import torch

from . import ops
from .engine import TowerLayout, round_up


def layout_x3(feature_size, hidden=5000, output_size=256):
    L = TowerLayout(feature_size, hidden, output_size)
    L.Fp, L.Hp, L.Dp = round_up(L.F, 256), round_up(L.H, 256), round_up(L.D, 256)
    L.sizes = (L.Fp * L.Hp, L.Hp, L.Hp * L.Dp, L.Dp)
    off = [0]
    for n in L.sizes[:-1]:
        off.append(off[-1] + n)
    L.offsets = tuple(off)
    L.numel = int(sum(L.sizes))
    return L


class TowerWorkspaceX3:
    def __init__(self, layout, n_rows, device, products=6, planes_in=True, backward=True, transposed=None,
                 fc2_single_pass=False, kint=None):
        L, R = layout, int(n_rows)
        if R % 128:
            raise ValueError("precision 'f32x3' needs a row count that is a multiple of 128 (got %d)" % R)
        if products not in (3, 6):
            raise ValueError("products must be 6 (fp32-equivalent) or 3 (16-bit operands)")
        self.layout, self.R, self.products = L, R, products
        bf = lambda *s: torch.zeros(s, dtype=torch.bfloat16, device=device)
        f32 = lambda *s: torch.zeros(s, dtype=torch.float32, device=device)
        if transposed is None:
            transposed = (os.environ.get("CDML_X3_TRANSPOSED") == "1" and backward and R % 256 == 0 and products == 6)
        if transposed and (R % 256 or not backward):
            raise ValueError("the transposed activation layout needs a training workspace with rows % 256 == 0")
        self.transposed = bool(transposed)
        maskbits = backward and not self.transposed and os.environ.get("CDML_X3_MASKBITS", "1") != "0"
        if kint is None:
            kint = os.environ.get("CDML_X3_KI", "0") == "1" and planes_in
        self.kint = bool(kint) and maskbits and products == 6 and R % 8 == 0
        self.xk = None
        self.x3 = bf(R, 3 * L.Fp)
        self.x_hat = self.x3 if planes_in else f32(R, L.Fp)
        self.h1 = bf(L.Hp, 3 * R) if self.transposed else bf(R, 3 * L.Hp)
        self.z, self.e = f32(R, L.Dp), f32(R, L.Dp)
        self.W1T, self.W2T, self.W2 = bf(L.Hp, 3 * L.Fp), bf(L.Dp, 3 * L.Hp), bf(L.Hp, 3 * L.Dp)
        q = products
        self.fc2_single_pass = bool(fc2_single_pass) and not backward and R // 256 >= 192
        self.slab_steps = None if backward else 120
        nb = 16 if self.fc2_single_pass else max(ops.gemm_bf16x3_workspace(False, R, L.Dp, L.Hp, q), 16)
        self.h1_bits = None
        if maskbits:
            self.h1_bits = torch.zeros((R, L.Hp // 8), dtype=torch.uint8, device=device)
        if backward:
            self.dz1 = bf(L.Hp, 3 * R) if self.transposed else (None if self.kint else bf(R, 3 * L.Hp))
            self.dz1k = torch.zeros(3 * R * L.Hp, dtype=torch.bfloat16, device=device) if self.kint else None
            self.de, self.dz2 = f32(R, L.Dp), f32(R, L.Dp)
            self.dz2_3 = bf(R, 3 * L.Dp)
            nb = max(nb, ops.gemm_bf16x3_workspace(True, L.Fp, L.Hp, R, q), ops.gemm_bf16x3_workspace(True, L.Hp, L.Dp, R, q))
            if L.Fp % 512 == 0:
                nb = max(nb, ops.gemm_bf16x3_workspace(True, L.Fp // 2, L.Hp, R, q))
            if self.transposed:
                self.xT = bf(L.Fp, 3 * R)
                self.dz2T = bf(L.Dp, 3 * R)
                nb = max(nb, ops.gemm_bf16x3_workspace(True, R, L.Dp, L.Hp, q),
                         ops.gemm_bf16x3_workspace(False, L.Fp, L.Hp, R, q), ops.gemm_bf16x3_workspace(False, L.Hp, L.Dp, R, q))
                if L.Fp % 512 == 0:
                    nb = max(nb, ops.gemm_bf16x3_workspace(False, L.Fp // 2, L.Hp, R, q))
        self.gemm_ws = torch.empty(nb // 4, dtype=torch.float32, device=device)
        self.tail_done = False

    def _sum_planes(self, t, width):
        return t[:, :width].float() + t[:, width:2 * width].float() + t[:, 2 * width:3 * width].float()

    def x_hat_f32(self):
        return self.x_hat if self.x_hat.dtype == torch.float32 else self._sum_planes(self.x_hat, self.layout.Fp)

    def dz1_f32(self):
        if self.transposed:
            return self._sum_planes(self.dz1, self.R).t().contiguous()
        if self.dz1 is None:
            v = self.dz1k.view(3, self.R // 8, self.layout.Hp, 8).permute(0, 1, 3, 2).reshape(3, self.R, self.layout.Hp)
            return v[0].float() + v[1].float() + v[2].float()
        return self._sum_planes(self.dz1, self.layout.Hp)

    def h1_f32(self):
        H, R = self.layout.Hp, self.R
        if self.transposed:
            return (self.h1[:, :R].float() + self.h1[:, R:2 * R].float() + self.h1[:, 2 * R:].float()).t().contiguous()
        return self.h1[:, :H].float() + self.h1[:, H:2 * H].float() + self.h1[:, 2 * H:].float()


def refresh_weights(p, ws):
    L = p.layout
    ops.split_f32_bf16x3(p.W1, ws.W1T, L.Fp, transpose=True)
    ops.split_f32_bf16x3(p.W2, ws.W2T, L.Hp, transpose=True)
    ops.split_f32_bf16x3(p.W2, ws.W2, L.Dp)
    if getattr(ws, "W1n", None) is not None:
        ops.split_f32_bf16x3(p.W1, ws.W1n, L.Hp)


def tower_forward(p, ws, normalize=True):
    L, R, q = p.layout, ws.R, ws.products
    if ws.x_hat.dtype == torch.float32:
        ops.split_f32_bf16x3(ws.x_hat, ws.x3, L.Fp)
    else:
        ws.x3 = ws.x_hat
    if ws.transposed:
        ops.gemm_bf16x3_nt(ops.BE_ROWBIAS_LRELU_X3, ws.W1T, L.Fp, ws.x3, L.Fp, ws.h1, L.Hp, R, L.Fp, products=q,
                           plane_c=R, bias=p.b1)
        ops.gemm_bf16x3_tn(ws.h1, R, ws.W2, L.Dp, ws.z, R, L.Dp, L.Hp, products=q, workspace=ws.gemm_ws, bias=p.b2)
    else:
        if getattr(ws, "h1_bits", None) is not None:
            ops.gemm_bf16x3_nt(ops.BE_BIAS_LRELU_X3_BITS, ws.x3, L.Fp, ws.W1T, L.Fp, ws.h1, R, L.Hp, L.Fp, products=q,
                               plane_c=L.Hp, bias=p.b1, aux=ws.h1_bits)
        else:
            ops.gemm_bf16x3_nt(ops.BE_BIAS_LRELU_X3, ws.x3, L.Fp, ws.W1T, L.Fp, ws.h1, R, L.Hp, L.Fp, products=q,
                               plane_c=L.Hp, bias=p.b1)
        ops.gemm_bf16x3_nt(ops.BE_BIAS_LRELU_F32, ws.h1, L.Hp, ws.W2T, L.Hp, ws.z, R, L.Dp, L.Hp, products=q,
                           bias=p.b2, workspace=None if getattr(ws, "fc2_single_pass", False) else ws.gemm_ws,
                           slab_steps=getattr(ws, "slab_steps", None))
    ws.tail_done = False
    ws.dz2_planes_done = False
    if normalize:
        ops.l2norm_fwd(ws.z, L.Dp, ws.e)
    return ws.e


def tower_backward(p, ws, after_w1=None, w1_chunks=1, after_w1_chunk=None):
    L, R, q = p.layout, ws.R, ws.products
    if not ws.tail_done:
        ops.l2norm_bwd(ws.z, ws.de, L.Dp, ws.dz2, lrelu_alpha=ops.LRELU_ALPHA)
    if not (ws.tail_done and getattr(ws, "dz2_planes_done", False)):
        ops.split_f32_bf16x3(ws.dz2, ws.dz2_3, L.Dp)
    T = ws.transposed
    if T:
        ops.split_f32_bf16x3(ws.dz2, ws.dz2T, R, transpose=True)
        w2 = lambda: ops.gemm_bf16x3_nt(ops.BE_F32, ws.h1, R, ws.dz2T, R, p.gW2, L.Hp, L.Dp, R, products=q,
                                        workspace=ws.gemm_ws, colsum=p.gb2)
    else:
        w2 = lambda: ops.gemm_bf16x3_tn(ws.h1, L.Hp, ws.dz2_3, L.Dp, p.gW2, L.Hp, L.Dp, R, products=q,
                                        workspace=ws.gemm_ws, colsum=p.gb2)
    single = after_w1 is None and after_w1_chunk is None
    if single:
        w2()
    if T:
        ops.gemm_bf16x3_nt(ops.BE_MASK_X3, ws.W2, L.Dp, ws.dz2_3, L.Dp, ws.dz1, L.Hp, R, L.Dp, products=q, plane_c=R,
                           aux=ws.h1)
        for pl in range(3):
            ops.transpose_to_bf16(ws.x3[:, pl * L.Fp:(pl + 1) * L.Fp], ws.xT[:, pl * R:(pl + 1) * R], R, L.Fp)
    else:
        kint = getattr(ws, "kint", False) and ws.xk is not None and getattr(ws, "h1_bits", None) is not None
        if getattr(ws, "kint", False) and not kint:
            raise RuntimeError("this workspace holds dz1 k8-interleaved only: it needs the gather's interleaved x_hat (ws.xk) and "
                               "the sign bitmask of h1 (CDML_X3_MASKBITS); build it with kint=False otherwise")
        if kint:
            ops.gemm_bf16x3_nt(ops.BE_MASKBITS_X3_KI, ws.dz2_3, L.Dp, ws.W2, L.Dp, ws.dz1k, R, L.Hp, L.Dp, products=q,
                               plane_c=R * L.Hp, aux=ws.h1_bits, ldc=L.Hp)
        elif getattr(ws, "h1_bits", None) is not None:
            ops.gemm_bf16x3_nt(ops.BE_MASKBITS_X3, ws.dz2_3, L.Dp, ws.W2, L.Dp, ws.dz1, R, L.Hp, L.Dp, products=q,
                               plane_c=L.Hp, aux=ws.h1_bits)
        else:
            ops.gemm_bf16x3_nt(ops.BE_MASK_X3, ws.dz2_3, L.Dp, ws.W2, L.Dp, ws.dz1, R, L.Hp, L.Dp, products=q, plane_c=L.Hp,
                               aux=ws.h1)
    rows = L.Fp // w1_chunks if w1_chunks > 1 else 0

    def dw1(lo, hi, db):
        if T:
            ops.gemm_bf16x3_nt(ops.BE_F32, ws.xT[lo:hi], R, ws.dz1, R, p.gW1[lo:hi], hi - lo, L.Hp, R, products=q,
                               workspace=ws.gemm_ws, colsum=db)
        elif getattr(ws, "kint", False):
            ops.gemm_bf16x3_tnk(ws.xk, L.Fp, lo, ws.dz1k, L.Hp, 0, p.gW1[lo:hi], hi - lo, L.Hp, R, workspace=ws.gemm_ws, colsum=db)
        else:
            ops.gemm_bf16x3_tn(ws.x3[:, lo:], L.Fp, ws.dz1, L.Hp, p.gW1[lo:hi], hi - lo, L.Hp, R, products=q,
                               workspace=ws.gemm_ws, colsum=db)
    if after_w1_chunk is not None and w1_chunks > 1 and rows * w1_chunks == L.Fp and rows % 256 == 0:
        for c in range(w1_chunks):
            last = c == w1_chunks - 1
            dw1(c * rows, (c + 1) * rows, p.gb1 if last else None)
            after_w1_chunk(c * rows * L.Hp, (c + 1) * rows * L.Hp + (L.Hp if last else 0))
    else:
        dw1(0, L.Fp, p.gb1)
        if after_w1_chunk is not None:
            after_w1_chunk(0, L.Fp * L.Hp + L.Hp)
    if after_w1 is not None:
        after_w1()
    if not single:
        w2()
    return p.grad
```

collaborative-deep-metric-learning_amd/ops.py:

```python
import ctypes as C

import torch

from ._lib import call, load_library

LRELU_ALPHA = 0.2


def _stream():
    return C.c_void_p(torch.cuda.current_stream().cuda_stream)


def _p(t, dtype=None):
    if t is None:
        return C.c_void_p(0)
    if not t.is_cuda:
        raise ValueError("cdml ops need device tensors (there is no CPU path)")
    if dtype is not None and t.dtype != dtype:
        raise ValueError(f"expected {dtype}, got {t.dtype}")
    return C.c_void_p(t.data_ptr())


def _mat(t, dtype=torch.float32):
    if t.dim() != 2 or t.stride(1) != 1:
# ... 192 lines not shown
    dxp, dxld = _mat(dx)
    if x_post is None:
        xpp, xpld = C.c_void_p(0), 0
    else:
        xpp, xpld = _mat(x_post)
    call("cdml_fc_bwd_data", dyp, dyld, wp, wld, xpp, xpld, alpha, M, K, N, dxp, dxld, _stream())
    return dx


def fc_bwd_weight_workspace(M, K, N):
    return int(load_library().cdml_fc_bwd_weight_workspace(M, K, N))


def fc_bwd_weight(x, dy, dW, db, workspace, M, K, N):
    xp, xld = _mat(x)
    dyp, dyld = _mat(dy)
    wp, wld = _mat(dW)
    call("cdml_fc_bwd_weight", xp, xld, dyp, dyld, M, K, N, wp, wld, _p(db, torch.float32),
         _p(workspace), workspace.numel() * workspace.element_size(), _stream())
    return dW, db


def fc_bwd_weight2_workspace(M, K1, N1, K2, N2):
    return int(load_library().cdml_fc_bwd_weight2_workspace(M, K1, N1, K2, N2))


def fc_bwd_weight2(x1, dy1, dW1, db1, K1, N1, x2, dy2, dW2, db2, K2, N2, M, workspace):
    a1, lda1 = _mat(x1)
    b1, ldb1 = _mat(dy1)
    c1, ldc1 = _mat(dW1)
    a2, lda2 = _mat(x2)
    b2, ldb2 = _mat(dy2)
    c2, ldc2 = _mat(dW2)
    call("cdml_fc_bwd_weight2", a1, lda1, b1, ldb1, K1, N1, c1, ldc1, _p(db1, torch.float32), a2, lda2, b2, ldb2,
         K2, N2, c2, ldc2, _p(db2, torch.float32), M, _p(workspace), workspace.numel() * workspace.element_size(),
         _stream())


def triplet_hinge(e, B, D, margin, pos, neg, hinge, stats=None, de=None):
    ep, eld = _mat(e)
    dep, deld = (C.c_void_p(0), 0) if de is None else _mat(de)
    call("cdml_triplet_hinge", ep, eld, B, D, margin, _p(pos), _p(neg), _p(hinge), _p(stats), dep,
         deld, _stream())


def triplet_hinge_inbatch(e, rows, shift, B, D, margin, pos, neg, hinge, valid=None, stats=None,
                          de=None):
    ep, eld = _mat(e)
    dep, deld = (C.c_void_p(0), 0) if de is None else _mat(de)
    call("cdml_triplet_hinge_inbatch", ep, eld, _p(rows, torch.int32), _p(shift, torch.int32), B, D,
         margin, _p(pos), _p(neg), _p(hinge), _p(valid, torch.uint8), _p(stats), dep, deld, _stream())


TICKET_WORDS = 128


def new_tickets(device):
    return torch.zeros(TICKET_WORDS, dtype=torch.int32, device=device)


def vnet_tail_workspace_floats(B, D):
    return int(load_library().cdml_vnet_tail_workspace(B, D)) // 4


def vnet_tail(mode, z, rows, shift, B, D, margin, e, pos, neg, hinge, dz2, valid=None, stats=None,
              dz2_bf16=None, var_ws=None, alpha=LRELU_ALPHA, plane_bf=0, h2_scale=0.0):
    zp, zld = _mat(z)
    ep, eld = _mat(e)
    dp, dld = _mat(dz2)
    bp, bld = (C.c_void_p(0), 0) if dz2_bf16 is None else _mat16(dz2_bf16)
    if h2_scale:
        call("cdml_vnet_tail_h2", mode, zp, zld, _p(rows, torch.int32), _p(shift, torch.int32), B, D, margin, alpha,
             ep, eld, _p(pos), _p(neg), _p(hinge), _p(valid, torch.uint8), dp, dld, bp, bld, plane_bf, float(h2_scale), _p(stats),
             _p(var_ws), _stream())
        return
    if plane_bf:
        call("cdml_vnet_tail_planes", mode, zp, zld, _p(rows, torch.int32), _p(shift, torch.int32), B, D, margin, alpha,
             ep, eld, _p(pos), _p(neg), _p(hinge), _p(valid, torch.uint8), dp, dld, bp, bld, plane_bf, _p(stats),
             _p(var_ws), _stream())
        return
    call("cdml_vnet_tail", mode, zp, zld, _p(rows, torch.int32), _p(shift, torch.int32), B, D, margin, alpha,
         ep, eld, _p(pos), _p(neg), _p(hinge), _p(valid, torch.uint8), dp, dld, bp, bld, _p(stats), _p(var_ws),
         _stream())


def semihard_select(S, e, rows, B, D, sqn_scratch, neg_row_out):
    sp, sld = _mat(S)
    ep, eld = _mat(e)
    call("cdml_semihard_select", sp, sld, ep, eld, _p(rows, torch.int32), B, D, _p(sqn_scratch),
         _p(neg_row_out, torch.int32), _stream())
    return neg_row_out


def semihard_mine_x3_workspace(B):
    return int(load_library().cdml_semihard_mine_x3_workspace(B))


def semihard_mine_x3(e, rows, B, D, e_planes, plane, sqn, dp, workspace, neg_row_out, z=None, h2_scale=0.0):
    ep, eld = _mat(e)
    pp, pld = _mat16(e_planes)
    if h2_scale:
        zp, zld = (C.c_void_p(0), 0) if z is None else _mat(z)
        call("cdml_semihard_mine_h2", zp, zld, ep, eld, _p(rows, torch.int32), B, D, pp, pld, plane, float(h2_scale), _p(sqn), _p(dp),
             _p(workspace), workspace.numel() * workspace.element_size(), _p(neg_row_out, torch.int32), _stream())
        return neg_row_out
    if z is not None:
        zp, zld = _mat(z)
        call("cdml_semihard_mine_x3_z", zp, zld, ep, eld, _p(rows, torch.int32), B, D, pp, pld, plane, _p(sqn), _p(dp),
             _p(workspace), workspace.numel() * workspace.element_size(), _p(neg_row_out, torch.int32), _stream())
        return neg_row_out
    call("cdml_semihard_mine_x3", ep, eld, _p(rows, torch.int32), B, D, pp, pld, plane, _p(sqn), _p(dp),
         _p(workspace), workspace.numel() * workspace.element_size(), _p(neg_row_out, torch.int32), _stream())
    return neg_row_out


def triplet_hinge_indexed(e, neg_row, B, D, margin, pos, neg, hinge, scale_scratch, stats=None, de=None, z=None, dz2=None,
                          dz2_bf16=None, plane_bf=0, lrelu_alpha=LRELU_ALPHA):
    ep, eld = _mat(e)
    dep, deld = (C.c_void_p(0), 0) if de is None else _mat(de)
    if z is None:
        call("cdml_triplet_hinge_indexed", ep, eld, _p(neg_row, torch.int32), B, D, margin, _p(pos), _p(neg),
             _p(hinge), _p(stats), _p(scale_scratch), dep, deld, _stream())
        return
    zp, zld = _mat(z)
    dzp, dzld = _mat(dz2)
    bp, bld = (C.c_void_p(0), 0) if dz2_bf16 is None else _mat16(dz2_bf16)
    call("cdml_triplet_hinge_indexed_tail", ep, eld, _p(neg_row, torch.int32), B, D, margin, _p(pos), _p(neg),
         _p(hinge), _p(stats), _p(scale_scratch), dep, deld, zp, zld, lrelu_alpha, dzp, dzld, bp, bld, plane_bf, _stream())


NPAIR_PRECISIONS = ("f32x3", "f32", "bf16")
NPAIR_FP32_PRECISIONS = ("f32x3", "f32")
NPAIR_TILE = {"f32x3": 256, "f32": 64, "bf16": 256}
_NPAIR_PRECISION_MSG = "the N-pair loss runs on precision 'f32x3', 'f32' or 'bf16', not %r"


def npair_workspace(B):
    return int(load_library().cdml_npair_workspace(int(B)))


def npair_stats(S, rows, B, temperature, symmetric, lse, stats, workspace):
    sp, sld = _mat(S)
    call("cdml_npair_stats", sp, sld, _p(rows, torch.int32), int(B), float(temperature), 1 if symmetric else 0, _p(lse),
         _p(stats), _p(workspace), workspace.numel() * workspace.element_size(), _stream())
    return lse, stats


def npair_grad_x3(S, rows, B, temperature, symmetric, lse, W_planes, plane):
    sp, sld = _mat(S)
    wp, wld = _mat16(W_planes)
    call("cdml_npair_grad_x3", sp, sld, _p(rows, torch.int32), int(B), float(temperature), 1 if symmetric else 0, _p(lse),
         wp, wld, int(plane), _stream())
    return W_planes


def npair_grad_f32(S, rows, B, temperature, symmetric, lse, W):
    sp, sld = _mat(S)
    wp, wld = _mat(W)
    call("cdml_npair_grad_f32", sp, sld, _p(rows, torch.int32), int(B), float(temperature), 1 if symmetric else 0, _p(lse),
         wp, wld, _stream())
    return W


def npair_operands_bf16(e, B, D, A, P, PT):
    ep, eld = _mat(e)
    ap, ald = _mat16(A)
# ... 1088 lines not shown

def _mat16(t):
    if t.dim() != 2 or t.stride(1) != 1 or t.element_size() != 2:
        raise ValueError("expected a 2-D 16-bit tensor with unit inner stride")
    return _p(t), t.stride(0)


def gemm_bf16_workspace(M, N, K):
    return int(load_library().cdml_gemm_bf16_workspace(M, N, K))


def gemm_bf16_nt(epilogue, A, B, C, M, N, K, bias=None, aux=None, alpha=LRELU_ALPHA, workspace=None):
    ap, ald = _mat16(A)
    bp, bld = _mat16(B)
    if C.dim() != 2 or C.stride(1) != 1:
        raise ValueError("C must be 2-D with unit inner stride")
    xld = aux.stride(0) if aux is not None else 0
    if aux is not None and (aux.dtype == torch.uint8) != (epilogue in (BE_BIAS_LRELU_BF16_BITS, BE_MASKBITS_BF16)):
        raise ValueError("epilogues 4 / 5 take a uint8 bitmask as aux, epilogue 2 bf16 values")
    call("cdml_gemm_bf16_nt", epilogue, ap, ald, bp, bld, M, N, K, _p(C), C.stride(0), _p(bias),
         _p(aux), xld, alpha, _p(workspace), 0 if workspace is None else workspace.numel() * workspace.element_size(),
         _stream())
    return C


def gemm_bf16_tn_supported(M, N, K, lda, ldb):
    return bool(load_library().cdml_gemm_bf16_tn_supported(M, N, K, lda, ldb))


def gemm_bf16_tn_workspace(M, N, K):
    return int(load_library().cdml_gemm_bf16_tn_workspace(M, N, K))


def gemm_bf16_tn(A, B, C, M, N, K, workspace=None, colsum=None):
    ap, ald = _mat16(A)
    bp, bld = _mat16(B)
    cp, cld = _mat(C)
    call("cdml_gemm_bf16_tn", ap, ald, bp, bld, M, N, K, cp, cld, _p(colsum, torch.float32), _p(workspace),
         0 if workspace is None else workspace.numel() * workspace.element_size(), _stream())
    return C


BE_BIAS_LRELU_X3, BE_MASK_X3, BE_ROWBIAS_LRELU_X3 = 6, 7, 8
BE_BIAS_LRELU_X3_BITS, BE_MASKBITS_X3 = 9, 10
BE_MASKBITS_X3_KI = 12


def split_f32_bf16x3(src, dst, plane, transpose=False):
    sp, sld = _mat(src)
    dp, dld = _mat16(dst)
    call("cdml_split_f32_bf16x3", sp, sld, src.shape[0], src.shape[1], dp, dld, plane, 1 if transpose else 0, _stream())
    return dst


def gemm_bf16x3_workspace(tn, M, N, K, products=6):
    return int(load_library().cdml_gemm_bf16x3_workspace(1 if tn else 0, M, N, K, products))


def gemm_bf16x3_nt(epilogue, A, plane_a, B, plane_b, C, M, N, K, products=6, plane_c=0, bias=None, aux=None,
                   alpha=LRELU_ALPHA, workspace=None, colsum=None, ldc=None, slab_steps=None):
    if slab_steps:
        lib = load_library()
        prev = lib.cdml_x3_slab_steps(int(slab_steps))
        try:
            return gemm_bf16x3_nt(epilogue, A, plane_a, B, plane_b, C, M, N, K, products=products, plane_c=plane_c, bias=bias,
                                  aux=aux, alpha=alpha, workspace=workspace, colsum=colsum, ldc=ldc)
        finally:
            lib.cdml_x3_slab_steps(prev)
    ap, ald = _mat16(A)
    bp, bld = _mat16(B)
    if epilogue == BE_MASKBITS_X3_KI:
        if ldc is None or not C.is_contiguous() or C.dtype != torch.bfloat16:
            raise ValueError("epilogue 12 writes a contiguous bf16 buffer and needs ldc (columns per row group)")
    elif C.dim() != 2 or C.stride(1) != 1:
        raise ValueError("C must be 2-D with unit inner stride")
    if aux is not None and (aux.dtype == torch.uint8) != (epilogue in (BE_BIAS_LRELU_X3_BITS, BE_MASKBITS_X3, BE_MASKBITS_X3_KI)):
        raise ValueError("epilogues 9 / 10 / 12 take a uint8 bitmask as aux, epilogue 7 bf16 values")
    call("cdml_gemm_bf16x3_nt", epilogue, ap, ald, plane_a, bp, bld, plane_b, M, N, K, products, _p(C), C.stride(0) if ldc is None else ldc,
         plane_c, _p(bias), _p(aux), aux.stride(0) if aux is not None else 0, alpha, _p(colsum, torch.float32),
         _p(workspace), 0 if workspace is None else workspace.numel() * workspace.element_size(), _stream())
    return C


def interleave8_bf16x3(src, plane_src, rows, cols, dst):
    sp, sld = _mat16(src)
    if dst.dtype != torch.bfloat16 or not dst.is_contiguous() or dst.numel() < 3 * rows * cols:
        raise ValueError("interleave8_bf16x3: dst must be a contiguous bf16 buffer of 3 * rows * cols elements")
    call("cdml_interleave8_bf16x3", sp, sld, plane_src, rows, cols, C.c_void_p(dst.data_ptr()), _stream())
    return dst


def gemm_bf16x3_tnk(A, ma, a_col0, B, nb, b_col0, out, M, N, K, workspace=None, colsum=None):
    cp, cld = _mat(out)
    ws, wb = (C.c_void_p(0), 0) if workspace is None else (C.c_void_p(workspace.data_ptr()), workspace.numel() * workspace.element_size())
    call("cdml_gemm_bf16x3_tnk", C.c_void_p(A.data_ptr()), ma, a_col0, C.c_void_p(B.data_ptr()), nb, b_col0, M, N, K, cp, cld,
         _p(colsum, torch.float32), ws, wb, _stream())
    return out


def gemm_bf16x3_tn(A, plane_a, B, plane_b, C, M, N, K, products=6, workspace=None, colsum=None, bias=None,
                   alpha=LRELU_ALPHA):
    ap, ald = _mat16(A)
    bp, bld = _mat16(B)
    cp, cld = _mat(C)
    call("cdml_gemm_bf16x3_tn", ap, ald, plane_a, bp, bld, plane_b, M, N, K, products, cp, cld, _p(bias), alpha,
         _p(colsum, torch.float32), _p(workspace),
         0 if workspace is None else workspace.numel() * workspace.element_size(), _stream())
    return C


def split_f32_f16x2(src, dst, plane, scale, transpose=False):
    sp, sld = _mat(src)
    dp, dld = _mat16(dst)
    call("cdml_split_f32_f16x2", sp, sld, src.shape[0], src.shape[1], dp, dld, plane, 1 if transpose else 0, float(scale), _stream())
    return dst


def gemm_f16x2_workspace(tn, M, N, K):
    return int(load_library().cdml_gemm_f16x2_workspace(1 if tn else 0, M, N, K))


def gemm_f16x2_nt(epilogue, A, plane_a, B, plane_b, C, M, N, K, out_scale, c_scale=1.0, plane_c=0, bias=None, aux=None,
                  alpha=LRELU_ALPHA, workspace=None, slab_steps=None):
    if slab_steps:
        lib = load_library()
        prev = lib.cdml_x3_slab_steps(int(slab_steps))
        try:
            return gemm_f16x2_nt(epilogue, A, plane_a, B, plane_b, C, M, N, K, out_scale, c_scale=c_scale, plane_c=plane_c,
                                 bias=bias, aux=aux, alpha=alpha, workspace=workspace)
        finally:
            lib.cdml_x3_slab_steps(prev)
    ap, ald = _mat16(A)
    bp, bld = _mat16(B)
    if C.dim() != 2 or C.stride(1) != 1:
        raise ValueError("C must be 2-D with unit inner stride")
    if aux is not None and (aux.dtype == torch.uint8) != (epilogue in (BE_BIAS_LRELU_X3_BITS, BE_MASKBITS_X3)):
        raise ValueError("epilogues 9 / 10 take a uint8 bitmask as aux, epilogue 7 16-bit values")
    call("cdml_gemm_f16x2_nt", epilogue, ap, ald, plane_a, bp, bld, plane_b, M, N, K, _p(C), C.stride(0), plane_c, _p(bias),
         _p(aux), aux.stride(0) if aux is not None else 0, alpha, float(out_scale), float(c_scale), _p(workspace),
         0 if workspace is None else workspace.numel() * workspace.element_size(), _stream())
    return C


def gemm_f16x2_tn(A, plane_a, B, plane_b, C, M, N, K, out_scale, workspace=None, colsum=None, colsum_scale=1.0):
    ap, ald = _mat16(A)
    bp, bld = _mat16(B)
    cp, cld = _mat(C)
    call("cdml_gemm_f16x2_tn", ap, ald, plane_a, bp, bld, plane_b, M, N, K, cp, cld, float(out_scale), _p(colsum, torch.float32),
         float(colsum_scale), _p(workspace), 0 if workspace is None else workspace.numel() * workspace.element_size(), _stream())
    return C


def gemm_bf16_tn2_workspace(M1, N1, M2, N2, K):
    return int(load_library().cdml_gemm_bf16_tn2_workspace(M1, N1, M2, N2, K))


def gemm_bf16_tn2(A1, B1, C1, M1, N1, A2, B2, C2, M2, N2, K, workspace, colsum1=None, colsum2=None):
    a1, lda1 = _mat16(A1)
    b1, ldb1 = _mat16(B1)
    c1, ldc1 = _mat(C1)
    a2, lda2 = _mat16(A2)
    b2, ldb2 = _mat16(B2)
    c2, ldc2 = _mat(C2)
    call("cdml_gemm_bf16_tn2", a1, lda1, b1, ldb1, M1, N1, c1, ldc1, _p(colsum1, torch.float32), a2, lda2, b2, ldb2,
         M2, N2, c2, ldc2, _p(colsum2, torch.float32), K, _p(workspace), workspace.numel() * workspace.element_size(),
         _stream())
# ... 184 lines not shown
```

collaborative-deep-metric-learning_amd/train.py:

```python
import logging
import os
import time

import torch

from . import engine, engine_bf16, engine_f16x2, engine_x3, ops
from .inputs import MODE_INBATCH, MODE_UNIFORM

_MODES = {"uniform": MODE_UNIFORM, "inbatch": MODE_INBATCH, "semihard": MODE_INBATCH, "npair": MODE_INBATCH}


def exponential_decay(base_lr, global_step, decay_steps, decay_rate, staircase=True):
    p = global_step / float(decay_steps)
    if staircase:
        p = float(int(p))
    return base_lr * (decay_rate ** p)


class TrainStep:
    GRAD_SYNC_MODES = ("bucketed", "two", "single")

    def __init__(self, table, pairs, batch_size, feature_size=None, output_size=256,
                 hidden_size=5000, margin=0.8, mode="uniform", optimizer="adam",
                 base_learning_rate=0.01, learning_rate_decay_examples=1000000,
# ... 104 lines not shown
                raise ValueError("memory_size must be a multiple of the batch (%d pairs) and of %d on precision %r (got %d)"
                                 % (int(batch_size), tile, precision, memory_size))
        if optimizer not in ("adam", "lars", "momentum"):
            raise ValueError("optimizer must be 'adam', 'lars' or 'momentum'")
        self.device = torch.device(device)
        if self.device.type == "cuda" and self.device.index is not None \
                and torch.cuda.current_device() != self.device.index:
            raise ValueError("TrainStep(device=%s) needs torch.cuda.set_device(%d) first (current device %d)"
                             % (self.device, self.device.index, torch.cuda.current_device()))
        self.table, self.pairs = table, pairs
        if pairs.numel():
            lo, hi = int(pairs.min().item()), int(pairs.max().item())
            if lo < 0 or hi >= table.n_rows_global:
                raise IndexError("co-watch pair ids span [%d, %d] but the catalogue has %d rows"
                                 % (lo, hi, table.n_rows_global))
        self.B = int(batch_size)
        self.mode = mode
        self.uniform_negatives = uniform_negatives
        self.sampler_mode = MODE_UNIFORM if uniform_negatives else _MODES[mode]
        self.rows_per_triplet = 3 if self.sampler_mode == MODE_UNIFORM else 2
        self.R = self.B * self.rows_per_triplet
        self.margin = float(margin)
        self.temperature, self.symmetric = float(temperature), bool(symmetric)
        self.seed = int(seed)
        self.optimizer = optimizer
        self.base_lr = float(base_learning_rate)
        self.decay_steps = learning_rate_decay_examples
        self.decay_rate = learning_rate_decay
        self.exchange, self.grad_sync = exchange, grad_sync
        if grad_sync_mode not in self.GRAD_SYNC_MODES:
            raise ValueError("grad_sync_mode must be one of %s" % (self.GRAD_SYNC_MODES,))
        self._grad_sync_mode = grad_sync_mode
        self.slot0 = int(slot0)
        self.batch_global = self.B if batch_global is None else int(batch_global)
        F = table.feature_size if feature_size is None else feature_size
        if precision in ("auto", None):
            if table.data.dtype == torch.float16:
                precision = "bf16"
            else:
                precision = "f32x3" if (self.B * self.rows_per_triplet) % 128 == 0 else "f32"
        if precision not in ("f32", "bf16", "f32x3", "f32x3-3", "f16x2"):
            raise ValueError("precision must be 'auto', 'f32', 'f32x3', 'f16x2' or 'bf16'")
        self.precision = precision
        self.bf16 = precision == "bf16"
        self.x3 = precision.startswith("f32x3")
        self.h2 = precision == "f16x2"
        if self.bf16 != (table.data.dtype == torch.float16):
            raise ValueError("precision 'bf16' goes with an fp16 FeatureTableF16, 'f32' / 'f32x3' with an fp32 table")
        if self.h2:
            if use_graph and (use_graph == "split" or exchange is not None or grad_sync is not None):
                raise ValueError("precision 'f16x2' replays from a hipGraph on one GPU only (its plane scales are kernel arguments "
                                 "baked into a capture: the check steps run eagerly and a moved scale re-captures, engine_f16x2.py)")
            self._h2_sig = None
            self.layout = engine_x3.layout_x3(F, hidden_size, output_size)
            self.params = engine.VNetParams(self.layout, self.device, weight_seed)
            self.ws = engine_f16x2.TowerWorkspaceH2(self.layout, self.R, self.device, planes_in=exchange is None)
        elif self.x3:
            self.layout = engine_x3.layout_x3(F, hidden_size, output_size)
            self.params = engine.VNetParams(self.layout, self.device, weight_seed)
            self.ws = engine_x3.TowerWorkspaceX3(self.layout, self.R, self.device, products=3 if precision.endswith("-3") else 6,
                                                 planes_in=True,
                                                 kint=None if (exchange is None and not train_table) else False)
            engine_x3.refresh_weights(self.params, self.ws)
        elif self.bf16:
            self.layout = engine_bf16.layout_bf16(F, hidden_size, output_size)
            self.params = engine.VNetParams(self.layout, self.device, weight_seed)
            self.ws = engine_bf16.TowerWorkspaceBF16(self.layout, self.R, self.device)
            engine_bf16.refresh_weights(self.params, self.ws)
        else:
            self.layout = engine.TowerLayout(F, hidden_size, output_size)
            self.params = engine.VNetParams(self.layout, self.device, weight_seed)
            self.ws = engine.TowerWorkspace(self.layout, self.R, self.device)
        dev, i32, f32 = self.device, torch.int32, torch.float32
        self.idx = torch.zeros(self.R, dtype=i32, device=dev)
        self.shift = torch.zeros(1, dtype=i32, device=dev)
        self.pos = torch.zeros(self.B, dtype=f32, device=dev)
        self.neg = torch.zeros(self.B, dtype=f32, device=dev)
        self.hinge = torch.zeros(self.B, dtype=f32, device=dev)
        self.valid = torch.ones(self.B, dtype=torch.uint8, device=dev)
        self.stats = torch.zeros(8, dtype=f32, device=dev)
        self.oob = torch.zeros(1, dtype=i32, device=dev)
        self.adam_tickets = ops.new_tickets(dev)
        self.var_ws = None
        if mode == "semihard":
            if self.B % 32:
                raise ValueError("semi-hard mining needs a batch that is a multiple of 32")
            self.mine_fused = ((precision == "f32x3" or self.h2) and (2 * self.B) % 256 == 0 and self.layout.Dp % 64 == 0
                               and os.environ.get("CDML_MINE_FUSED", "1") != "0")
            if self.mine_fused:
                Dp = self.layout.Dp
                self.e3 = (torch.zeros((2 * self.B, 2 * Dp), dtype=torch.float16, device=dev) if self.h2
                           else torch.zeros((2 * self.B, 3 * Dp), dtype=torch.bfloat16, device=dev))
                self.dp = torch.zeros(self.B, dtype=f32, device=dev)
                self.mine_ws = torch.zeros(ops.semihard_mine_x3_workspace(self.B) // 4, dtype=f32, device=dev)
            else:
                self.S = torch.zeros((self.B, 2 * self.B), dtype=f32, device=dev)
            self.sqn = torch.zeros(2 * self.B, dtype=f32, device=dev)
            self.neg_row = torch.zeros(self.B, dtype=i32, device=dev)
            self.scale = torch.zeros(self.B, dtype=f32, device=dev)
        self.memory_size, self.memory_start = memory_size, memory_start
        self.npair_sync, self.npair_dp = npair_sync, None
        self.npair_memory = None
        self.npair_mixed = None
        if uniform_negatives:
            self.npair_mixed = ops.NPairMixed(self.B, self.layout.Dp, precision, dev, memory_size, memory_start)
            self.npair_memory = self.npair_mixed.ring
        elif mode == "npair" and npair_sync is not None:
            self.npair_dp = ops.NPairDP(self.B, self.B * npair_sync.world, self.layout.Dp, precision, dev)
        elif mode == "npair":
            self.npair_ws = ops.NPairWorkspace(self.B, self.layout.Dp, precision, dev, in_batch=not memory_size)
            if memory_size:
                self.npair_memory = ops.NPairMemory(memory_size, self.B, self.layout.Dp, precision, dev, start=memory_start)
        self.npair_logq = None
        if logq is not None:
            self.npair_logq = (ops.LogQEstimator(table.n_rows_global, self.B, logq_alpha, logq_init_gap, dev) if logq_stream
                               else ops.LogQTable(logq, dev))
        self.uniform_lq = ops.uniform_logq(self.npair_logq, uniform_logq) if uniform_negatives else 0.0
        self.neg_lists = None
        self.hard_fraction = float(hard_fraction)
        if negative_lists is not None:
            self.neg_lists = negative_lists.to(dev).contiguous().clone()
            self.kind = torch.zeros(self.B, dtype=i32, device=dev)
        self.step_dev = torch.zeros(1, dtype=torch.int64, device=dev)
        self.lr_dev = torch.full((1,), self.base_lr, dtype=f32, device=dev)
        self._lr_host = self.base_lr
        self.global_step = 0
        n = self.layout.numel
        if optimizer == "adam":
            self.m = torch.zeros(n, dtype=f32, device=dev)
            self.v = torch.zeros(n, dtype=f32, device=dev)
        else:
            self.acc = torch.zeros(n, dtype=f32, device=dev)
        self.lars_scratch = torch.zeros(max(ops.lars_scratch_floats(), ops.lars_multi_scratch_floats()), dtype=f32,
                                        device=dev)
        self.clip_gradient_norm = float(clip_gradient_norm)
        self.reg_scale = float(regularization_penalty) * float(l2_penalty)
        self.l2_penalty = float(l2_penalty)
        self.grad_norms = torch.zeros((4, 2), dtype=f32, device=dev)
        self.train_table = bool(train_table)
        if self.train_table:
            if self.bf16 or optimizer != "adam" or precision == "f32x3-3":
                raise ValueError("train_table goes with an fp32 catalogue (precision 'f32x3' or 'f32') and the Adam optimizer")
            if self.x3:
                if getattr(self.ws, "transposed", False) or self.ws.dz1 is None:
                    raise ValueError("train_table needs the row-major activation layout of the f32x3 path")
                self.ws.W1n = torch.zeros((self.layout.Fp, 3 * self.layout.Hp), dtype=torch.bfloat16, device=dev)
                engine_x3.refresh_weights(self.params, self.ws)
            elif self.h2:
                self.ws.W1n = torch.zeros((self.layout.Fp, 2 * self.layout.Hp), dtype=torch.float16, device=dev)
            self.tab_m = torch.zeros_like(table.data)
            self.tab_v = torch.zeros_like(table.data)
            self.tab_head = torch.full((table.n_rows,), -1, dtype=i32, device=dev)
            self.tab_next = torch.zeros(self.R, dtype=i32, device=dev)
            self.dxh = torch.zeros((self.R, self.layout.Fp), dtype=f32, device=dev)
            prefetch = False
            if grad_sync is not None and exchange is None:
                raise ValueError("train_table with grad_sync needs a row-sharded table (exchange): "
                                 "replicated trainable tables would diverge between ranks")
        kint = self.x3 and getattr(self.ws, "kint", False)
        if gather_ahead in ("auto", None, 0):
            row_bytes = self.ws.x_hat.shape[-1] * self.ws.x_hat.element_size() * (2 if kint else 1)
            target = 230e6 if self.bf16 else 300e6
            gather_ahead = min(4, max(1, int(round(target / (self.R * row_bytes)))))
        self.gather_ahead = max(1, int(gather_ahead))
        if exchange is not None or self.train_table or self.neg_lists is not None:
            self.gather_ahead = 1
# ... 122 lines not shown
            if t == 0 or self._filled != t:
                self.prefetch.launch(b, lambda: self._fill(b, t))
            self.prefetch.acquire(b)
            self.ws.x_hat, self.idx, self.shift = self._x[b], self._idx[b], self._shift[b]
            return
        if self.neg_lists is not None:
            ops.sample_gather_listed(self.pairs, self.seed, None, self.B, self.table.data, self.table.feature_size,
                                     self.neg_lists, self.hard_fraction, self.idx, self.ws.x_hat, kind_out=self.kind,
                                     slot0=self.slot0, batch_global=self.batch_global, step_dev=self.step_dev,
                                     oob_flag=self.oob,
                                     x_ki=self.ws.xk if (self.x3 and getattr(self.ws, "kint", False)) else None)
        elif self.exchange is None:
            ops.sample_gather(m, self.pairs, self.seed, None, self.B, self.table.data,
                              self.table.feature_size, self.idx, self.ws.x_hat,
                              shift_out=self.shift, slot0=self.slot0,
                              batch_global=self.batch_global, step_dev=self.step_dev, oob_flag=self.oob,
                              x_ki=self.ws.xk if (self.x3 and getattr(self.ws, "kint", False)) else None)
        else:
            if m == MODE_UNIFORM:
                ops.sample_uniform(self.pairs, self.table.n_rows_global, self.seed, None, self.B,
                                   self.idx, slot0=self.slot0, batch_global=self.batch_global,
                                   step_dev=self.step_dev)
            else:
                ops.sample_inbatch(self.pairs, self.seed, None, self.B, self.idx, self.shift,
                                   slot0=self.slot0, batch_global=self.batch_global,
                                   step_dev=self.step_dev)
            self.exchange.gather(self.table, self.idx, self.ws.x_hat)

    def set_negative_lists(self, lists):
        if self.neg_lists is None:
            raise ValueError("this step has no negative lists (TrainStep(negative_lists=...))")
        lists = torch.as_tensor(lists)
        if lists.dtype != torch.int32 or tuple(lists.shape) != tuple(self.neg_lists.shape):
            raise ValueError("negative lists must stay int32 %s, got %s %s"
                             % (tuple(self.neg_lists.shape), lists.dtype, tuple(lists.shape)))
        self.neg_lists.copy_(lists)

    def hard_share(self):
        if self.neg_lists is None:
            raise ValueError("this step has no negative lists (TrainStep(negative_lists=...))")
        return float(self.kind.sum().item()) / self.B

    def refresh_negative_lists(self, k, skip_top=0, drop_partners=True):
        from . import hardneg
        from .predict import Prediction
        if self.neg_lists is None:
            raise ValueError("this step has no negative lists (TrainStep(negative_lists=...))")
        if hardneg.list_width(k) != self.neg_lists.shape[1]:
            raise ValueError("k = %d gives lists of width %d, this step holds lists of width %d"
                             % (k, hardneg.list_width(k), self.neg_lists.shape[1]))
        if getattr(self, "_list_predictor", None) is None:
            self._list_predictor = Prediction(params=self.params, precision="bf16" if self.bf16 else "f32x3" if self.x3 else "f32")
        emb = self._list_predictor.embed_table(self.table, 16384)
        lists = hardneg.mine_lists(emb, k, skip_top=skip_top, pairs=self.pairs if drop_partners else None, device=self.device)
        self.set_negative_lists(lists)
        return lists

    def enable_variance(self, on=True):
        L = self.layout
        self.var_ws = (torch.zeros(ops.vnet_tail_workspace_floats(self.B, L.Dp), dtype=torch.float32,
                                   device=self.device) if on else None)
        self._graphs = {}

    def variance(self):
        if self.var_ws is None:
            raise RuntimeError("call enable_variance() before the step")
        return float(self.stats[4].item()) * self.layout.Dp / self.layout.D

    def forward_loss(self, with_grad=True):
        due = self.h2 and self.ws.scales.due(self.global_step)
        if due:
            engine_f16x2.observe_weights(self.params, self.ws)
        self._forward_loss(with_grad)
        if due and with_grad:
            engine_f16x2.observe_gradients(self.params, self.ws)

    def _forward_loss(self, with_grad=True):
        fused = with_grad and self.mode not in ("semihard", "npair")
        mine_norm = (self.mode == "semihard" and getattr(self, "mine_fused", False)
                     and os.environ.get("CDML_MINE_NORM", "1") != "0")
        if self.h2:
            engine_f16x2.tower_forward(self.params, self.ws, normalize=not (fused or mine_norm))
        elif self.x3:
            engine_x3.tower_forward(self.params, self.ws, normalize=not (fused or mine_norm))
        elif self.bf16:
            engine_bf16.tower_forward(self.params, self.ws, normalize=not fused)
        else:
            engine.tower_forward(self.params, self.ws, normalize=not fused)
        L = self.layout
        if fused:
            ops.vnet_tail(0 if self.mode == "uniform" else 1, self.ws.z, self.idx, self.shift, self.B, L.Dp,
                          self.margin, self.ws.e, self.pos, self.neg, self.hinge, self.ws.dz2, valid=self.valid,
                          stats=self.stats, var_ws=self.var_ws,
                          dz2_bf16=self.ws.dz2_bf if self.bf16 else self.ws.dz2_3 if self.x3 else self.ws.dz2_2 if self.h2 else None,
                          plane_bf=L.Dp if (self.x3 or self.h2) else 0, h2_scale=self.ws.scales.dz2 if self.h2 else 0.0)
            self.ws.tail_done = True
            self.ws.dz2_planes_done = self.x3 or self.h2
            return
        de = self.ws.de if with_grad else None
        if self.npair_mixed is not None:
            ops.npair_mixed_loss(self.ws.e, self.idx, self.B, L.Dp, self.temperature, self.symmetric, self.precision, de=de,
                                 stats=self.stats, ws=self.npair_mixed, step=0, step_dev=self.step_dev, logq=self.npair_logq,
                                 lq_u=self.uniform_lq)
        elif self.npair_dp is not None:
            if self.prefetch is not None:
                self.prefetch.wait_ready(1 - self.global_step % 2)
            ops.npair_dp_loss(self.ws.e, self.idx, self.B, L.Dp, self.temperature, self.symmetric, self.precision, de=de,
                              stats=self.stats, ws=self.npair_dp, sync=self.npair_sync)
        elif self.mode == "npair":
            ops.npair_loss(self.ws.e, self.idx, self.B, L.Dp, self.temperature, self.symmetric, self.precision, de=de,
                           stats=self.stats, ws=self.npair_ws, memory=self.npair_memory, step=0, step_dev=self.step_dev,
                           logq=self.npair_logq)
        elif self.mode == "uniform":
            ops.triplet_hinge(self.ws.e, self.B, L.Dp, self.margin, self.pos, self.neg, self.hinge,
                              self.stats, de)
        elif self.mode == "semihard":
            e = self.ws.e
            if self.mine_fused:
                ops.semihard_mine_x3(e, self.idx, self.B, L.Dp, self.e3, L.Dp, self.sqn, self.dp, self.mine_ws, self.neg_row,
                                     z=self.ws.z if mine_norm else None, h2_scale=engine_f16x2.X_SCALE if self.h2 else 0.0)
            else:
                ops.fc_bwd_data(e[0::2], e, None, self.S, self.B, 2 * self.B, L.Dp)
                ops.semihard_select(self.S, e, self.idx, self.B, L.Dp, self.sqn, self.neg_row)
            if with_grad and os.environ.get("CDML_INDEXED_TAIL", "1") != "0":
                ops.triplet_hinge_indexed(e, self.neg_row, self.B, L.Dp, self.margin, self.pos, self.neg, self.hinge,
                                          self.scale, self.stats, de, z=self.ws.z, dz2=self.ws.dz2,
                                          dz2_bf16=self.ws.dz2_bf if self.bf16 else self.ws.dz2_3 if self.x3 else None,
                                          plane_bf=L.Dp if self.x3 else 0)
                self.ws.tail_done = True
                self.ws.dz2_planes_done = self.x3
            else:
                ops.triplet_hinge_indexed(e, self.neg_row, self.B, L.Dp, self.margin, self.pos, self.neg,
                                          self.hinge, self.scale, self.stats, de)
        else:
            ops.triplet_hinge_inbatch(self.ws.e, self.idx, self.shift, self.B, L.Dp, self.margin,
                                      self.pos, self.neg, self.hinge, self.valid, self.stats, de)

    def backward(self, after_w1=None):
        if self.h2:
            engine_f16x2.tower_backward(self.params, self.ws, after_w1=after_w1)
        elif self.x3:
            engine_x3.tower_backward(self.params, self.ws, after_w1=after_w1)
        elif self.bf16:
            engine_bf16.tower_backward(self.params, self.ws, after_w1=after_w1)
        else:
            engine.tower_backward(self.params, self.ws, after_w1=after_w1)

    def update_table(self):
        L, p, t = self.layout, self.params, self.table
        if self.h2:
            sc = self.ws.scales
            ops.gemm_f16x2_nt(ops.BE_F32, self.ws.dz1, L.Hp, self.ws.W1n, L.Hp, self.dxh, self.R, L.Fp, L.Hp,
                              1.0 / (sc.dz1 * sc.w1))
        elif self.x3:
            ops.gemm_bf16x3_nt(ops.BE_F32, self.ws.dz1, L.Hp, self.ws.W1n, L.Hp, self.dxh, self.R, L.Fp, L.Hp,
                               products=self.ws.products)
        else:
            ops.fc_bwd_data(self.ws.dz1, p.W1, None, self.dxh, self.R, L.Fp, L.Hp)
        idx, rows = self.idx, self.dxh
        if self.exchange is not None:
            idx, rows = self.exchange.scatter_back(self.dxh)
            if idx.numel() == 0:
                return
            if self.tab_next.numel() < idx.numel():
                self.tab_next = torch.zeros(idx.numel(), dtype=torch.int32, device=self.device)
        world = self.grad_sync.world if self.grad_sync is not None else 1
        ops.table_adam_rows(t.data, t.row0, t.feature_size, idx, rows, self.tab_m, self.tab_v,
                            self.tab_head, self.tab_next, 0.0, 1, lr_dev=self.lr_dev, t_dev=self.step_dev,
                            grad_scale=1.0 / world)

    def reg_loss(self):
        n = self.grad_norms.cpu()
# ... 473 lines not shown
```

Measured before the change: 3.110 million.

## Fuse split-K slab reduction and bias-LReLU of fc2 into the triplet loss tail

When the x3 second-layer GEMM is split into K slabs, the slab-sum kernel is skipped. The loss tail reads the slabs directly, sums them, applies bias and leaky-ReLU, writes z, and computes the triplet loss in one kernel. A last-block ticket also folds the stats and variance finalisation into that kernel, removing separate launches. This cuts a round trip of z through memory and one or two launches, at the cost of more loads per tail row (every split for each of the 3 or 5 rows it reads) and atomic-scope stores.

```diff
diff --git a/__graft_entry__.py b/__graft_entry__.py
--- a/__graft_entry__.py
+++ b/__graft_entry__.py
@@ -110,7 +110,7 @@
     lib = _lib.load_library()
     assert lib.cdml_version() >= 1000
     for name in list(_lib.SIGNATURES) + list(_lib.SIGNATURES_MIXED) + list(_lib.SIGNATURES_DP) + list(_lib.SIGNATURES_BF16) \
-            + list(_lib.SIGNATURES_HARDNEG):
+            + list(_lib.SIGNATURES_HARDNEG) + list(_lib.SIGNATURES_TAIL):
         getattr(lib, name)
     assert lib.cdml_build_id().decode() == "CDML_BUILD_ID=" + sid
     print("[build] ok:", LIB, "version", lib.cdml_version(), lib.cdml_build_id().decode())
diff --git a/collaborative-deep-metric-learning_amd/_lib.py b/collaborative-deep-metric-learning_amd/_lib.py
--- a/collaborative-deep-metric-learning_amd/_lib.py
+++ b/collaborative-deep-metric-learning_amd/_lib.py
@@ -216,6 +216,13 @@
     "cdml_npair_memory_push_bf16": (_i, [_p, _i64, _p, _i, _i, _u64, _p, _i64, _i, _p, _i64, _p, _p, _i64, _p, _i64, _p]),
 }
 
+SIGNATURES_TAIL = {
+    "cdml_gemm_bf16x3_nt_slab_count": (_i, [_i, _i, _i, _i]),
+    "cdml_gemm_bf16x3_nt_slabs": (_i, [_p, _i64, _i64, _p, _i64, _i64, _i, _i, _i, _i, _p, _sz, _p, _p, _p]),
+    "cdml_vnet_tail_slabs": (_i, [_i, _p, _i64, _i, _p, _p, _i64, _p, _p, _i, _i, _f, _f, _p, _i64, _p, _p, _p, _p, _p, _i64,
+                                  _p, _i64, _i64, _p, _p, _i, _p]),
+}
+
 SIGNATURES_HARDNEG = {
     "cdml_sample_listed": (_i, [_p, _i64, _i64, _u64, _u64, _p, _i, _i64, _i64, _p, _i64, _i, _u64, _p, _p, _p]),
     "cdml_sample_gather_listed": (_i, [_p, _i64, _u64, _u64, _p, _i, _i64, _i64, _p, _i64, _i64, _i, _p, _i64, _i, _u64,
@@ -241,7 +248,8 @@
     import torch
     lib = C.CDLL(path)
     for name, (res, args) in (list(SIGNATURES.items()) + list(SIGNATURES_MIXED.items()) + list(SIGNATURES_DP.items())
-                               + list(SIGNATURES_BF16.items()) + list(SIGNATURES_HARDNEG.items())):
+                               + list(SIGNATURES_BF16.items()) + list(SIGNATURES_HARDNEG.items())
+                               + list(SIGNATURES_TAIL.items())):
         fn = getattr(lib, name)
         fn.restype = res
         fn.argtypes = args
diff --git a/collaborative-deep-metric-learning_amd/csrc/gemm_bf16x3.hip b/collaborative-deep-metric-learning_amd/csrc/gemm_bf16x3.hip
--- a/collaborative-deep-metric-learning_amd/csrc/gemm_bf16x3.hip
+++ b/collaborative-deep-metric-learning_amd/csrc/gemm_bf16x3.hip
@@ -1,4 +1,5 @@
 #include "gemm_bf16.h"
+#include "../../include/cdml_tail_slabs.h"
 #include <stdlib.h>
 
 namespace cdml {
@@ -272,7 +273,8 @@
                            const uint16_t *B, int64_t ldb, int64_t plane_b, int M, int N, int K, int products, void *C,
                            int64_t ldc, int64_t plane_c, const float *bias, const uint16_t *aux,
                            int64_t ldaux, float alpha, float *colsum, void *workspace,
-                           size_t workspace_bytes, cdml_stream_t stream) {
+                           size_t workspace_bytes, cdml_stream_t stream, int *slabs_only = nullptr,
+                           int64_t *slab_stride_out = nullptr) {
   CDML_REQUIRE(A && B && C && M > 0 && N > 0 && K > 0, CDML_E_BADARG, "gemm_bf16x3_nt: bad argument");
   const int np1 = f16 ? 1 : 2;
   CDML_REQUIRE(!f16 || (products == 3 && epilogue != BE_MASKBITS_X3_KI && epilogue != BE_ROWBIAS_LRELU_X3 && !colsum &&
@@ -347,6 +349,8 @@
     g.colsum_partial = reinterpret_cast<float *>(static_cast<char *>(workspace) + slab_bytes);
   }
   int rc;
+  CDML_REQUIRE(!slabs_only || splits > 1, CDML_E_UNSUPPORTED,
+               "gemm_bf16x3_nt_slabs: this product is not split into K slabs (cdml_gemm_bf16x3_nt_slab_count = 1): use cdml_gemm_bf16x3_nt");
   if (splits == 1) {
     rc = launch(epilogue, 1);
   } else {
@@ -355,6 +359,11 @@
     g.C = workspace; g.ldc = N;
     rc = launch(BE_F32, splits);
     if (rc) return rc;
+    if (slabs_only) {
+      *slabs_only = splits;
+      *slab_stride_out = g.slab_stride;
+      return CDML_OK;
+    }
     const int sb = grid1d((int64_t)M * N / 4), cb = colsum ? (N + 15) / 16 : 0;
     hipLaunchKernelGGL(k_x3_sum_slabs, dim3(sb + cb), dim3(kThreads), 0, s,
                        static_cast<const float *>(workspace), g.slab_stride, splits, M, N,
@@ -376,6 +385,25 @@
                                    size_t workspace_bytes, cdml_stream_t stream) {
   return gemm_x3_nt_impl(false, 1.0f, 1.0f, epilogue, A, lda, plane_a, B, ldb, plane_b, M, N, K, products, C, ldc, plane_c, bias, aux,
                          ldaux, alpha, colsum, workspace, workspace_bytes, stream);
+}
+
+extern "C" int cdml_gemm_bf16x3_nt_slab_count(int M, int N, int K, int products) {
+  if (M <= 0 || N <= 0 || K <= 0 || (products != 3 && products != 6) || K % 64 || N % 256) return 0;
+  const int ktiles = products * (K / 64);
+  int splits = x3_nt_splits(N, ktiles, (M + 255) / 256), per = ktiles;
+  if (splits > 1) x3_split_geometry(ktiles, splits, 6, per, splits);
+  return splits;
+}
+
+extern "C" int cdml_gemm_bf16x3_nt_slabs(const uint16_t *A, int64_t lda, int64_t plane_a, const uint16_t *B, int64_t ldb,
+                                         int64_t plane_b, int M, int N, int K, int products, void *workspace,
+                                         size_t workspace_bytes, int *splits_out, int64_t *slab_stride_out,
+                                         cdml_stream_t stream) {
+  CDML_REQUIRE(workspace && splits_out && slab_stride_out, CDML_E_BADARG,
+               "gemm_bf16x3_nt_slabs: the workspace and both outputs are required");
+  return gemm_x3_nt_impl(false, 1.0f, 1.0f, BE_BIAS_LRELU_F32, A, lda, plane_a, B, ldb, plane_b, M, N, K, products, workspace, N, 0,
+                         static_cast<const float *>(workspace), nullptr, 0, 0.f, nullptr, workspace, workspace_bytes, stream,
+                         splits_out, slab_stride_out);
 }
 
 extern "C" int cdml_gemm_f16x2_nt(int epilogue, const uint16_t *A, int64_t lda, int64_t plane_a, const uint16_t *B,
diff --git a/collaborative-deep-metric-learning_amd/csrc/loss.hip b/collaborative-deep-metric-learning_amd/csrc/loss.hip
--- a/collaborative-deep-metric-learning_amd/csrc/loss.hip
+++ b/collaborative-deep-metric-learning_amd/csrc/loss.hip
@@ -1,4 +1,6 @@
+#include <stdlib.h>
 #include "common.h"
+#include "../../include/cdml_tail_slabs.h"
 
 namespace cdml {
 namespace {
@@ -176,7 +178,97 @@
     inv = 1.0f / sqrtf(fmaxf(ss, kL2Eps));
   }
   __device__ __forceinline__ float4 e(int c) const { return mul4(v[c], inv); }
+  template <bool PLAIN_ZW = false>
+  __device__ __forceinline__ void set(const float4 (&x)[NCH]) {
+    static_assert(NCH == 1, "the slab form holds one 16-B chunk per lane and row");
+    v[0] = x[0];
+    const float xy = __builtin_fmaf(x[0].x, x[0].x, x[0].y * x[0].y);
+    float s;
+    if (PLAIN_ZW) {
+#pragma clang fp contract(off)
+      const float zz = x[0].z * x[0].z, ww = x[0].w * x[0].w;
+      s = ww + (zz + xy);
+    } else {
+      s = __builtin_fmaf(x[0].w, x[0].w, __builtin_fmaf(x[0].z, x[0].z, xy));
+    }
+    ss = wave_sum(s);
+    inv = 1.0f / sqrtf(fmaxf(ss, kL2Eps));
+  }
 };
+
+struct TailSlabs {
+  const float *slabs;
+  int64_t stride;
+  int splits;
+  const float *bias;
+  float *z;
+  int64_t ldz;
+  uint32_t *ticket;
+  float *stats;
+};
+
+template <int NCH, int NR>
+__device__ __forceinline__ void tail_slab_rows(const TailSlabs &S, const int64_t (&row)[NR], int D, int nq, int lane,
+                                               float alpha, float4 (&v)[NR][NCH]) {
+  const float4 zero = make_float4(0.f, 0.f, 0.f, 0.f);
+#pragma unroll
+  for (int u = 0; u < NR; ++u)
+#pragma unroll
+    for (int c = 0; c < NCH; ++c) {
+      const int q = lane + kWave * c;
+      v[u][c] = (q < nq) ? ld4(S.slabs + row[u] * D, q) : zero;
+    }
+#pragma unroll 4
+  for (int z = 1; z < S.splits; ++z) {
+    const float *sz = S.slabs + (int64_t)z * S.stride;
+    float4 t[NR][NCH];
+#pragma unroll
+    for (int u = 0; u < NR; ++u)
+#pragma unroll
+      for (int c = 0; c < NCH; ++c) {
+        const int q = lane + kWave * c;
+        t[u][c] = (q < nq) ? ld4(sz + row[u] * D, q) : zero;
+      }
+#pragma unroll
+    for (int u = 0; u < NR; ++u)
+#pragma unroll
+      for (int c = 0; c < NCH; ++c) {
+        v[u][c].x += t[u][c].x; v[u][c].y += t[u][c].y; v[u][c].z += t[u][c].z; v[u][c].w += t[u][c].w;
+      }
+  }
+#pragma unroll
+  for (int c = 0; c < NCH; ++c) {
+    const int q = lane + kWave * c;
+    const float4 b = (q < nq) ? ld4(S.bias, q) : zero;
+#pragma unroll
+    for (int u = 0; u < NR; ++u) {
+      float4 s = v[u][c];
+      s.x += b.x; s.y += b.y; s.z += b.z; s.w += b.w;
+      s.x = fmaxf(s.x, s.x * alpha); s.y = fmaxf(s.y, s.y * alpha);
+      s.z = fmaxf(s.z, s.z * alpha); s.w = fmaxf(s.w, s.w * alpha);
+      using f32x4 = __attribute__((ext_vector_type(4))) float;
+      f32x4 o = {s.x, s.y, s.z, s.w};
+      asm volatile("" : "+v"(o));
+      v[u][c] = make_float4(o.x, o.y, o.z, o.w);
+    }
+  }
+}
+
+template <int NCH>
+__device__ __forceinline__ void tail_store_z(const float4 (&x)[NCH], float *zr, int nq, int lane) {
+#pragma unroll
+  for (int c = 0; c < NCH; ++c) {
+    const int q = lane + kWave * c;
+    if (q < nq) st4(zr, q, x[c]);
+  }
+}
+
+__device__ __forceinline__ void st_shared(float *p, float v) {
+  __hip_atomic_store(p, v, __ATOMIC_RELAXED, __HIP_MEMORY_SCOPE_AGENT);
+}
+__device__ __forceinline__ float ld_shared(const float *p) {
+  return __hip_atomic_load(p, __ATOMIC_RELAXED, __HIP_MEMORY_SCOPE_AGENT);
+}
 
 template <int NCH>
 __device__ __forceinline__ void tail_dist(const TailRow<NCH> &a, const TailRow<NCH> &p, const TailRow<NCH> &n,
@@ -258,14 +350,20 @@
   }
 }
 
-template <int MODE, int NCH>
+template <bool SHARED>
+__device__ __forceinline__ float tail_word(const float *p) { return SHARED ? ld_shared(p) : *p; }
+
+__device__ void tail_finish_last_block(uint32_t *ticket, const float *pos, const float *neg, const float *hinge, int B, int D,
+                                       const float *var_ws, float *stats);
+
+template <int MODE, int NCH, bool SLABS>
 __global__ void __launch_bounds__(kThreads)
 k_vnet_tail(const float *__restrict__ z, int64_t ldz, const int32_t *__restrict__ rows,
             const int32_t *__restrict__ shift_p, int B, int D, float margin, float alpha,
             float *__restrict__ e, int64_t lde, float *__restrict__ pos_o, float *__restrict__ neg_o,
             float *__restrict__ hinge_o, uint8_t *__restrict__ valid_o, float *__restrict__ dz2,
             int64_t lddz, uint16_t *__restrict__ dz2_bf, int64_t ldbf, float *__restrict__ var_ws,
-            int64_t plane_bf, float h2_scale) {
+            int64_t plane_bf, float h2_scale, TailSlabs S) {
   __shared__ __attribute__((aligned(16))) float s_red[kWavesPerBlock][8];
   extern __shared__ __attribute__((aligned(16))) float s_col[];
   const int lane = threadIdx.x & (kWave - 1);
@@ -277,6 +375,7 @@
   float tsq = 0.f;
 #pragma unroll
   for (int c = 0; c < NCH; ++c) csum[c] = make_float4(0.f, 0.f, 0.f, 0.f);
+  auto put = [](float *p, float v) { if (SLABS) st_shared(p, v); else *p = v; };
   for (int i = blockIdx.x * kWavesPerBlock + wave; i < B; i += gridDim.x * kWavesPerBlock) {
     TailRow<NCH> A, P, N;
     float4 ga[NCH], gp[NCH];
@@ -285,9 +384,18 @@
     float pos, neg;
     if (MODE == 0) {
       ra = 3 * (int64_t)i; rp = ra + 1;
-      A.load(z + ra * ldz, nq, lane);
-      P.load(z + rp * ldz, nq, lane);
-      N.load(z + (ra + 2) * ldz, nq, lane);
+      if constexpr (SLABS) {
+        const int64_t r3[3] = {ra, rp, ra + 2};
+        float4 x[3][NCH];
+        tail_slab_rows<NCH, 3>(S, r3, D, nq, lane, alpha, x);
+#pragma unroll
+        for (int u = 0; u < 3; ++u) tail_store_z<NCH>(x[u], S.z + r3[u] * S.ldz, nq, lane);
+        A.set(x[0]); P.set(x[1]); N.template set<true>(x[2]);
+      } else {
+        A.load(z + ra * ldz, nq, lane);
+        P.load(z + rp * ldz, nq, lane);
+        N.load(z + (ra + 2) * ldz, nq, lane);
+      }
       tail_dist<NCH>(A, P, N, pos, neg);
       const float t = pos - neg + margin;
       const float s = (t >= 0.f) ? two_over_b : 0.f;
@@ -299,7 +407,7 @@
         gp[c] = mul4(sub4(vp, va), s);
         gn[c] = mul4(sub4(va, vn), s);
       }
-      if (lane == 0) { pos_o[i] = pos; neg_o[i] = neg; hinge_o[i] = fmaxf(t, 0.f); }
+      if (lane == 0) { put(pos_o + i, pos); put(neg_o + i, neg); put(hinge_o + i, fmaxf(t, 0.f)); }
       tail_store_row<NCH>(N, gn, alpha, e + (ra + 2) * lde, dz2 + (ra + 2) * lddz,
                           dz2_bf ? dz2_bf + (ra + 2) * ldbf : nullptr, nq, lane, plane_bf, h2_scale);
     } else {
@@ -310,11 +418,20 @@
       valid_i = (vn_id != va_id) && (vn_id != vp_id);
       const bool valid_k = (vp_id != rows[2 * k]) && (vp_id != rows[2 * k + 1]);
       TailRow<NCH> AK, PK;
-      A.load(z + ra * ldz, nq, lane);
-      P.load(z + rp * ldz, nq, lane);
-      N.load(z + (int64_t)(2 * j + 1) * ldz, nq, lane);
-      AK.load(z + (int64_t)(2 * k) * ldz, nq, lane);
-      PK.load(z + (int64_t)(2 * k + 1) * ldz, nq, lane);
+      if constexpr (SLABS) {
+        const int64_t r5[5] = {ra, rp, 2 * (int64_t)j + 1, 2 * (int64_t)k, 2 * (int64_t)k + 1};
+        float4 x[5][NCH];
+        tail_slab_rows<NCH, 5>(S, r5, D, nq, lane, alpha, x);
+        tail_store_z<NCH>(x[0], S.z + ra * S.ldz, nq, lane);
+        tail_store_z<NCH>(x[1], S.z + rp * S.ldz, nq, lane);
+        A.set(x[0]); P.set(x[1]); N.set(x[2]); AK.set(x[3]); PK.set(x[4]);
+      } else {
+        A.load(z + ra * ldz, nq, lane);
+        P.load(z + rp * ldz, nq, lane);
+        N.load(z + (int64_t)(2 * j + 1) * ldz, nq, lane);
+        AK.load(z + (int64_t)(2 * k) * ldz, nq, lane);
+        PK.load(z + (int64_t)(2 * k + 1) * ldz, nq, lane);
+      }
       tail_dist<NCH>(A, P, N, pos, neg);
       float posk, negk;
       tail_dist<NCH>(AK, PK, P, posk, negk);
@@ -330,8 +447,8 @@
         gp[c] = make_float4(g1.x + g2.x, g1.y + g2.y, g1.z + g2.z, g1.w + g2.w);
       }
       if (lane == 0) {
-        pos_o[i] = pos; neg_o[i] = neg;
-        hinge_o[i] = valid_i ? fmaxf(t, 0.f) : 0.f;
+        put(pos_o + i, pos); put(neg_o + i, neg);
+        put(hinge_o + i, valid_i ? fmaxf(t, 0.f) : 0.f);
         if (valid_o) valid_o[i] = valid_i ? 1 : 0;
       }
     }
@@ -347,42 +464,45 @@
       }
     }
   }
-  if (!var_ws) return;
-  float *mine = s_col + wave * D;
-#pragma unroll
-  for (int c = 0; c < NCH; ++c) {
-    const int q = lane + kWave * c;
-    if (q < nq) st4(mine, q, csum[c]);
-  }
-  tsq = wave_sum(tsq);
-  if (lane == 0) s_red[wave][0] = tsq;
-  __syncthreads();
-  float *out = var_ws + (int64_t)blockIdx.x * (D + 4);
-  for (int d = threadIdx.x; d < D; d += kThreads) {
-    float v = 0.f;
-    for (int w = 0; w < kWavesPerBlock; ++w) v += s_col[w * D + d];
-    out[d] = v;
-  }
-  if (threadIdx.x == 0) {
-    float v = 0.f;
-    for (int w = 0; w < kWavesPerBlock; ++w) v += s_red[w][0];
-    out[D] = v;
-  }
-}
-
-__global__ void __launch_bounds__(kThreads)
-k_tail_var_final(const float *__restrict__ var_ws, int nb, int B, int D, float *__restrict__ stats) {
+  if (!SLABS && !var_ws) return;
+  if (var_ws) {
+    float *mine = s_col + wave * D;
+#pragma unroll
+    for (int c = 0; c < NCH; ++c) {
+      const int q = lane + kWave * c;
+      if (q < nq) st4(mine, q, csum[c]);
+    }
+    tsq = wave_sum(tsq);
+    if (lane == 0) s_red[wave][0] = tsq;
+    __syncthreads();
+    float *out = var_ws + (int64_t)blockIdx.x * (D + 4);
+    for (int d = threadIdx.x; d < D; d += kThreads) {
+      float v = 0.f;
+      for (int w = 0; w < kWavesPerBlock; ++w) v += s_col[w * D + d];
+      put(out + d, v);
+    }
+    if (threadIdx.x == 0) {
+      float v = 0.f;
+      for (int w = 0; w < kWavesPerBlock; ++w) v += s_red[w][0];
+      put(out + D, v);
+    }
+  }
+  if (SLABS) tail_finish_last_block(S.ticket, pos_o, neg_o, hinge_o, B, D, var_ws, S.stats);
+}
+
+template <bool SHARED>
+__device__ __forceinline__ void tail_var_final(const float *var_ws, int nb, int B, int D, float *stats) {
   __shared__ double s_v[kWavesPerBlock];
   const int lane = threadIdx.x & (kWave - 1), wave = threadIdx.x >> 6;
   const double n_rows = 3.0 * (double)B;
   double vsum = 0.0;
   for (int d = threadIdx.x; d < D; d += kThreads) {
     double col = 0.0;
-    for (int b = 0; b < nb; ++b) col += (double)var_ws[(int64_t)b * (D + 4) + d];
+    for (int b = 0; b < nb; ++b) col += (double)tail_word<SHARED>(var_ws + (int64_t)b * (D + 4) + d);
     const double mean = col / n_rows;
     vsum -= n_rows * mean * mean;
   }
-  for (int b = threadIdx.x; b < nb; b += kThreads) vsum += (double)var_ws[(int64_t)b * (D + 4) + D];
+  for (int b = threadIdx.x; b < nb; b += kThreads) vsum += (double)tail_word<SHARED>(var_ws + (int64_t)b * (D + 4) + D);
 #pragma unroll
   for (int off = 32; off > 0; off >>= 1) vsum += __shfl_xor(vsum, off, 64);
   if (lane == 0) s_v[wave] = vsum;
@@ -392,6 +512,57 @@
     for (int w = 0; w < kWavesPerBlock; ++w) v += s_v[w];
     stats[4] = (float)(v / (n_rows * (double)D));
   }
+}
+
+__global__ void __launch_bounds__(kThreads)
+k_tail_var_final(const float *__restrict__ var_ws, int nb, int B, int D, float *__restrict__ stats) {
+  tail_var_final<false>(var_ws, nb, B, D, stats);
+}
+
+__device__ void tail_finish_last_block(uint32_t *ticket, const float *pos, const float *neg, const float *hinge, int B, int D,
+                                       const float *var_ws, float *stats) {
+  __shared__ int s_last;
+  __shared__ float s_st[4][1024 / kWave];
+  asm volatile("s_waitcnt vmcnt(0)" ::: "memory");
+  __syncthreads();
+  if (threadIdx.x == 0) {
+    const uint32_t t = __hip_atomic_fetch_add(ticket, 1u, __ATOMIC_RELAXED, __HIP_MEMORY_SCOPE_AGENT);
+    const int last = t == gridDim.x - 1;
+    if (last) {
+      __hip_atomic_store(ticket, 0u, __ATOMIC_RELAXED, __HIP_MEMORY_SCOPE_AGENT);
+      __builtin_amdgcn_fence(__ATOMIC_ACQUIRE, "agent");
+      asm volatile("s_waitcnt vmcnt(0)" ::: "memory");
+    }
+    s_last = last;
+  }
+  __syncthreads();
+  if (!s_last) return;
+  const int lane = threadIdx.x & (kWave - 1), wave = threadIdx.x >> 6;
+  constexpr int kVirt = 1024 / kThreads;
+#pragma unroll
+  for (int u = 0; u < kVirt; ++u) {
+    const int vwave = wave + kWavesPerBlock * u;
+    float acc[4] = {0.f, 0.f, 0.f, 0.f};
+    for (int i = vwave * kWave + lane; i < B; i += 1024) {
+      const float h = ld_shared(hinge + i);
+      acc[0] += h;
+      acc[1] += ld_shared(pos + i);
+      acc[2] += ld_shared(neg + i);
+      acc[3] += (h > 0.f) ? 1.f : 0.f;
+    }
+#pragma unroll
+    for (int c = 0; c < 4; ++c) {
+      const float v = wave_sum(acc[c]);
+      if (lane == 0) s_st[c][vwave] = v;
+    }
+  }
+  __syncthreads();
+  if (threadIdx.x < 4) {
+    float v = 0.f;
+    for (int w = 0; w < 1024 / kWave; ++w) v += s_st[threadIdx.x][w];
+    stats[threadIdx.x] = v / (float)B;
+  }
+  if (var_ws) tail_var_final<true>(var_ws, gridDim.x, B, D, stats);
 }
 
 __global__ void __launch_bounds__(kThreads)
@@ -883,9 +1054,15 @@
 
 constexpr int kTailVarBlocks = 256;
 
+static int tail_slab_blocks() {
+  const char *e = getenv("CDML_TAIL_SLAB_BLOCKS");
+  const int n = e ? atoi(e) : 0;
+  return n >= 1 ? (n > kNumCU * 8 ? kNumCU * 8 : n) : kNumCU * 4;
+}
+
 extern "C" size_t cdml_vnet_tail_workspace(int B, int D) {
   if (B <= 0 || D <= 0) return 0;
-  return (size_t)kTailVarBlocks * (size_t)(D + 4) * sizeof(float);
+  return ((size_t)kTailVarBlocks * (size_t)(D + 4) + 1) * sizeof(float);
 }
 
 static int vnet_tail_impl(int mode, const float *z, int64_t ldz, const int32_t *rows,
@@ -893,14 +1070,14 @@
                           float *e, int64_t lde, float *pos, float *neg, float *hinge,
                           uint8_t *valid_out, float *dz2, int64_t lddz2, uint16_t *dz2_bf16,
                           int64_t ldbf, int64_t plane_bf, float *stats, float *var_ws, cdml_stream_t stream,
-                          float h2_scale = 0.f) {
+                          float h2_scale = 0.f, const TailSlabs *slabs = nullptr) {
   CDML_REQUIRE(mode == 0 || mode == 1, CDML_E_BADARG, "vnet_tail: mode must be 0 (a,p,n rows) or 1 (in-batch)");
   CDML_REQUIRE(B >= (mode == 1 ? 2 : 1) && D > 0 && pos && neg && hinge, CDML_E_BADARG, "vnet_tail: bad argument");
   CDML_REQUIRE(mode == 0 || (rows && shift), CDML_E_BADARG, "vnet_tail: in-batch mode needs rows and shift");
   CDML_REQUIRE(!var_ws || stats, CDML_E_BADARG, "vnet_tail: the variance is written to stats[4]");
   CDML_REQUIRE(D <= 1024, CDML_E_UNSUPPORTED, "vnet_tail: embedding size %d > 1024", D);
   int rc;
-  if ((rc = check_rows("vnet_tail z", z, ldz, D))) return rc;
+  if ((rc = check_rows("vnet_tail z", slabs ? slabs->z : z, slabs ? slabs->ldz : ldz, D))) return rc;
   if ((rc = check_rows("vnet_tail e", e, lde, D))) return rc;
   if ((rc = check_rows("vnet_tail dz2", dz2, lddz2, D))) return rc;
   CDML_REQUIRE(!dz2_bf16 || (ldbf >= D && (ldbf & 3) == 0 && (reinterpret_cast<uintptr_t>(dz2_bf16) & 7) == 0),
@@ -909,17 +1086,24 @@
                CDML_E_ALIGN, "vnet_tail: planes need plane >= D (a multiple of 4) and a leading dimension >= 2 plane + D (fp16 planes: plane + D)");
   int grid = grid_rows(B);
   if (var_ws && grid > kTailVarBlocks) grid = kTailVarBlocks;
+  if (slabs && !var_ws && grid > tail_slab_blocks()) grid = tail_slab_blocks();
   const size_t lds = var_ws ? (size_t)kWavesPerBlock * D * sizeof(float) : 0;
   const int nch = ((D >> 2) + kWave - 1) / kWave;
-#define CDML_LAUNCH_TAIL(M, N)                                                                       \
-  hipLaunchKernelGGL((k_vnet_tail<M, N>), dim3(grid), dim3(kThreads), lds, (hipStream_t)stream, z, ldz, \
-                     rows, shift, B, D, margin, lrelu_alpha, e, lde, pos, neg, hinge, valid_out, dz2,  \
-                     lddz2, dz2_bf16, ldbf, var_ws, plane_bf, h2_scale)
-  if (mode == 0) {
-    if (nch <= 1) CDML_LAUNCH_TAIL(0, 1); else if (nch <= 2) CDML_LAUNCH_TAIL(0, 2); else CDML_LAUNCH_TAIL(0, 4);
-  } else {
-    if (nch <= 1) CDML_LAUNCH_TAIL(1, 1); else if (nch <= 2) CDML_LAUNCH_TAIL(1, 2); else CDML_LAUNCH_TAIL(1, 4);
-  }
+#define CDML_LAUNCH_TAIL(M, N, SL)                                                                            \
+  hipLaunchKernelGGL((k_vnet_tail<M, N, SL>), dim3(grid), dim3(kThreads), lds, (hipStream_t)stream, z, ldz,     \
+                     rows, shift, B, D, margin, lrelu_alpha, e, lde, pos, neg, hinge, valid_out, dz2,           \
+                     lddz2, dz2_bf16, ldbf, var_ws, plane_bf, h2_scale, SL ? *slabs : TailSlabs{})
+#define CDML_LAUNCH_TAIL_N(M, SL)                                                                               \
+  do {                                                                                                          \
+    if (nch <= 1) CDML_LAUNCH_TAIL(M, 1, SL); else if (nch <= 2) CDML_LAUNCH_TAIL(M, 2, SL); else CDML_LAUNCH_TAIL(M, 4, SL); \
+  } while (0)
+  if (slabs) {
+    CDML_REQUIRE(nch == 1, CDML_E_UNSUPPORTED, "vnet_tail_slabs: embedding size %d > 256", D);
+    if (mode == 0) CDML_LAUNCH_TAIL(0, 1, true); else CDML_LAUNCH_TAIL(1, 1, true);
+    return check_launch("vnet_tail_slabs");
+  }
+  if (mode == 0) CDML_LAUNCH_TAIL_N(0, false); else CDML_LAUNCH_TAIL_N(1, false);
+#undef CDML_LAUNCH_TAIL_N
 #undef CDML_LAUNCH_TAIL
   if ((rc = check_launch("vnet_tail"))) return rc;
   if (stats) {
@@ -951,6 +1135,27 @@
   CDML_REQUIRE(dz2_planes && plane_bf > 0, CDML_E_BADARG, "vnet_tail_planes: the plane buffer and its plane stride are required");
   return vnet_tail_impl(mode, z, ldz, rows, shift, B, D, margin, lrelu_alpha, e, lde, pos, neg, hinge, valid_out, dz2, lddz2,
                         dz2_planes, ldbf, plane_bf, stats, var_ws, stream);
+}
+
+extern "C" int cdml_vnet_tail_slabs(int mode, const float *slabs, int64_t slab_stride, int splits, const float *bias,
+                                    float *z, int64_t ldz, const int32_t *rows, const int32_t *shift, int B, int D,
+                                    float margin, float lrelu_alpha, float *e, int64_t lde, float *pos, float *neg,
+                                    float *hinge, uint8_t *valid_out, float *dz2, int64_t lddz2, uint16_t *dz2_planes,
+                                    int64_t ldbf, int64_t plane_bf, float *stats, float *tail_ws, int want_var,
+                                    cdml_stream_t stream) {
+  CDML_REQUIRE(slabs && bias && stats && tail_ws && aligned16(slabs) && aligned16(bias) && aligned16(tail_ws), CDML_E_BADARG,
+               "vnet_tail_slabs: slabs, bias, stats and the workspace are required (16-B aligned)");
+  CDML_REQUIRE(B > 0 && D > 0 && (D & 3) == 0 && splits >= 1 && splits <= 16, CDML_E_BADARG, "vnet_tail_slabs: bad shape or slab count");
+  const int64_t n_rows = (int64_t)(mode == 0 ? 3 : 2) * B;
+  CDML_REQUIRE(splits == 1 || (slab_stride >= n_rows * D && (slab_stride & 3) == 0), CDML_E_BADARG,
+               "vnet_tail_slabs: slabs of %lld rows x %d need a stride >= %lld (a multiple of 4)", (long long)n_rows, D,
+               (long long)(n_rows * D));
+  CDML_REQUIRE(lrelu_alpha >= 0.f, CDML_E_BADARG, "vnet_tail_slabs: the output layer's leaky-relu slope is required");
+  CDML_REQUIRE(!dz2_planes || plane_bf > 0, CDML_E_BADARG, "vnet_tail_slabs: the plane buffer goes with its plane stride");
+  TailSlabs S{slabs, slab_stride, splits, bias, z, ldz,
+              reinterpret_cast<uint32_t *>(tail_ws + (size_t)kTailVarBlocks * (size_t)(D + 4)), stats};
+  return vnet_tail_impl(mode, nullptr, 0, rows, shift, B, D, margin, lrelu_alpha, e, lde, pos, neg, hinge, valid_out, dz2, lddz2,
+                        dz2_planes, ldbf, dz2_planes ? plane_bf : 0, stats, want_var ? tail_ws : nullptr, stream, 0.f, &S);
 }
 
 extern "C" int cdml_vnet_tail_h2(int mode, const float *z, int64_t ldz, const int32_t *rows,
diff --git a/collaborative-deep-metric-learning_amd/engine_x3.py b/collaborative-deep-metric-learning_amd/engine_x3.py
--- a/collaborative-deep-metric-learning_amd/engine_x3.py
+++ b/collaborative-deep-metric-learning_amd/engine_x3.py
@@ -68,6 +68,7 @@
                     nb = max(nb, ops.gemm_bf16x3_workspace(False, L.Fp // 2, L.Hp, R, q))
         self.gemm_ws = torch.empty(nb // 4, dtype=torch.float32, device=device)
         self.tail_done = False
+        self.fc2_slabs = None
 
     def _sum_planes(self, t, width):
         return t[:, :width].float() + t[:, width:2 * width].float() + t[:, 2 * width:3 * width].float()
@@ -99,7 +100,7 @@
         ops.split_f32_bf16x3(p.W1, ws.W1n, L.Hp)
 
 
-def tower_forward(p, ws, normalize=True):
+def tower_forward(p, ws, normalize=True, fc2_slabs=False):
     L, R, q = p.layout, ws.R, ws.products
     if ws.x_hat.dtype == torch.float32:
         ops.split_f32_bf16x3(ws.x_hat, ws.x3, L.Fp)
@@ -116,9 +117,16 @@
         else:
             ops.gemm_bf16x3_nt(ops.BE_BIAS_LRELU_X3, ws.x3, L.Fp, ws.W1T, L.Fp, ws.h1, R, L.Hp, L.Fp, products=q,
                                plane_c=L.Hp, bias=p.b1)
-        ops.gemm_bf16x3_nt(ops.BE_BIAS_LRELU_F32, ws.h1, L.Hp, ws.W2T, L.Hp, ws.z, R, L.Dp, L.Hp, products=q,
-                           bias=p.b2, workspace=None if getattr(ws, "fc2_single_pass", False) else ws.gemm_ws,
-                           slab_steps=getattr(ws, "slab_steps", None))
+        ws.fc2_slabs = None
+        if fc2_slabs:
+            if normalize or ws.fc2_single_pass:
+                raise ValueError("fc2_slabs leaves z to the loss tail: no l2-normalise here, no single-pass second layer")
+            ws.fc2_slabs = ops.gemm_bf16x3_nt_slabs(ws.h1, L.Hp, ws.W2T, L.Hp, R, L.Dp, L.Hp, ws.gemm_ws, products=q,
+                                                    slab_steps=ws.slab_steps)
+        else:
+            ops.gemm_bf16x3_nt(ops.BE_BIAS_LRELU_F32, ws.h1, L.Hp, ws.W2T, L.Hp, ws.z, R, L.Dp, L.Hp, products=q,
+                               bias=p.b2, workspace=None if getattr(ws, "fc2_single_pass", False) else ws.gemm_ws,
+                               slab_steps=getattr(ws, "slab_steps", None))
     ws.tail_done = False
     ws.dz2_planes_done = False
     if normalize:
diff --git a/collaborative-deep-metric-learning_amd/ops.py b/collaborative-deep-metric-learning_amd/ops.py
--- a/collaborative-deep-metric-learning_amd/ops.py
+++ b/collaborative-deep-metric-learning_amd/ops.py
@@ -298,6 +298,19 @@
     call("cdml_vnet_tail", mode, zp, zld, _p(rows, torch.int32), _p(shift, torch.int32), B, D, margin, alpha,
          ep, eld, _p(pos), _p(neg), _p(hinge), _p(valid, torch.uint8), dp, dld, bp, bld, _p(stats), _p(var_ws),
          _stream())
+
+
+def vnet_tail_slabs(mode, slabs, slab_stride, splits, bias, z, rows, shift, B, D, margin, e, pos, neg, hinge, dz2, stats,
+                    tail_ws, valid=None, dz2_planes=None, plane_bf=0, want_var=False, alpha=LRELU_ALPHA):
+    zp, zld = _mat(z)
+    ep, eld = _mat(e)
+    dp, dld = _mat(dz2)
+    bp, bld = (C.c_void_p(0), 0) if dz2_planes is None else _mat16(dz2_planes)
+    if tail_ws.numel() < vnet_tail_workspace_floats(B, D):
+        raise ValueError("vnet_tail_slabs: tail_ws holds %d floats, needs %d" % (tail_ws.numel(), vnet_tail_workspace_floats(B, D)))
+    call("cdml_vnet_tail_slabs", mode, _p(slabs), slab_stride, splits, _p(bias), zp, zld, _p(rows, torch.int32),
+         _p(shift, torch.int32), B, D, margin, alpha, ep, eld, _p(pos), _p(neg), _p(hinge), _p(valid, torch.uint8), dp, dld,
+         bp, bld, plane_bf, _p(stats), _p(tail_ws), 1 if want_var else 0, _stream())
 
 
 def semihard_select(S, e, rows, B, D, sqn_scratch, neg_row_out):
@@ -1552,6 +1565,31 @@
     return C
 
 
+def _with_slab_steps(slab_steps, fn):
+    if not slab_steps:
+        return fn()
+    lib = load_library()
+    prev = lib.cdml_x3_slab_steps(int(slab_steps))
+    try:
+        return fn()
+    finally:
+        lib.cdml_x3_slab_steps(prev)
+
+
+def gemm_bf16x3_nt_slab_count(M, N, K, products=6, slab_steps=None):
+    return _with_slab_steps(slab_steps, lambda: int(load_library().cdml_gemm_bf16x3_nt_slab_count(M, N, K, products)))
+
+
+def gemm_bf16x3_nt_slabs(A, plane_a, B, plane_b, M, N, K, workspace, products=6, slab_steps=None):
+    ap, ald = _mat16(A)
+    bp, bld = _mat16(B)
+    splits, stride = C.c_int(0), C.c_int64(0)
+    _with_slab_steps(slab_steps, lambda: call("cdml_gemm_bf16x3_nt_slabs", ap, ald, plane_a, bp, bld, plane_b, M, N, K, products,
+                                              _p(workspace), workspace.numel() * workspace.element_size(), C.byref(splits),
+                                              C.byref(stride), _stream()))
+    return splits.value, stride.value
+
+
 def interleave8_bf16x3(src, plane_src, rows, cols, dst):
     sp, sld = _mat16(src)
     if dst.dtype != torch.bfloat16 or not dst.is_contiguous() or dst.numel() < 3 * rows * cols:
diff --git a/collaborative-deep-metric-learning_amd/train.py b/collaborative-deep-metric-learning_amd/train.py
--- a/collaborative-deep-metric-learning_amd/train.py
+++ b/collaborative-deep-metric-learning_amd/train.py
@@ -210,6 +210,13 @@
         self.oob = torch.zeros(1, dtype=i32, device=dev)
         self.adam_tickets = ops.new_tickets(dev)
         self.var_ws = None
+        self.slab_tail = (self.x3 and mode in ("uniform", "inbatch") and exchange is None and grad_sync is None
+                          and not self.ws.transposed and not self.ws.fc2_single_pass
+                          and os.environ.get("CDML_TAIL_SLABS", "1") != "0"
+                          and ops.gemm_bf16x3_nt_slab_count(self.R, self.layout.Dp, self.layout.Hp, self.ws.products,
+                                                            slab_steps=self.ws.slab_steps) > 1)
+        self.tail_ws = (torch.zeros(ops.vnet_tail_workspace_floats(self.B, self.layout.Dp), dtype=f32, device=dev)
+                        if self.slab_tail else None)
         if mode == "semihard":
             if self.B % 32:
                 raise ValueError("semi-hard mining needs a batch that is a multiple of 32")
@@ -498,12 +505,22 @@
         if self.h2:
             engine_f16x2.tower_forward(self.params, self.ws, normalize=not (fused or mine_norm))
         elif self.x3:
-            engine_x3.tower_forward(self.params, self.ws, normalize=not (fused or mine_norm))
+            engine_x3.tower_forward(self.params, self.ws, normalize=not (fused or mine_norm),
+                                    fc2_slabs=fused and self.slab_tail)
         elif self.bf16:
             engine_bf16.tower_forward(self.params, self.ws, normalize=not fused)
         else:
             engine.tower_forward(self.params, self.ws, normalize=not fused)
         L = self.layout
+        if fused and self.x3 and self.ws.fc2_slabs:
+            splits, stride = self.ws.fc2_slabs
+            ops.vnet_tail_slabs(0 if self.mode == "uniform" else 1, self.ws.gemm_ws, stride, splits, self.params.b2, self.ws.z,
+                                self.idx, self.shift, self.B, L.Dp, self.margin, self.ws.e, self.pos, self.neg, self.hinge,
+                                self.ws.dz2, self.stats, self.var_ws if self.var_ws is not None else self.tail_ws,
+                                valid=self.valid, dz2_planes=self.ws.dz2_3, plane_bf=L.Dp, want_var=self.var_ws is not None)
+            self.ws.tail_done = True
+            self.ws.dz2_planes_done = True
+            return
         if fused:
             ops.vnet_tail(0 if self.mode == "uniform" else 1, self.ws.z, self.idx, self.shift, self.B, L.Dp,
                           self.margin, self.ws.e, self.pos, self.neg, self.hinge, self.ws.dz2, valid=self.valid,
diff --git a/include/cdml_tail_slabs.h b/include/cdml_tail_slabs.h
--- /dev/null
+++ b/include/cdml_tail_slabs.h
@@ -0,0 +1,24 @@
+#ifndef CDML_TAIL_SLABS_H_
+#define CDML_TAIL_SLABS_H_
+
+#include "cdml.h"
+
+#ifdef __cplusplus
+extern "C" {
+#endif
+
+int cdml_gemm_bf16x3_nt_slab_count(int M, int N, int K, int products);
+int cdml_gemm_bf16x3_nt_slabs(const uint16_t *A, int64_t lda, int64_t plane_a, const uint16_t *B, int64_t ldb,
+                              int64_t plane_b, int M, int N, int K, int products, void *workspace,
+                              size_t workspace_bytes, int *splits_out, int64_t *slab_stride_out, cdml_stream_t stream);
+int cdml_vnet_tail_slabs(int mode, const float *slabs, int64_t slab_stride, int splits, const float *bias, float *z,
+                         int64_t ldz, const int32_t *rows, const int32_t *shift, int B, int D, float margin,
+                         float lrelu_alpha, float *e, int64_t lde, float *pos, float *neg, float *hinge,
+                         uint8_t *valid_out, float *dz2, int64_t lddz2, uint16_t *dz2_planes, int64_t ldbf,
+                         int64_t plane_bf, float *stats, float *tail_ws, int want_var, cdml_stream_t stream);
+
+#ifdef __cplusplus
+}
+#endif
+
+#endif
```

Measured after the change: 3.100 million. Within noise of the previous version (-0.3%).
